# ExaScience/elprep

Measured on AMD Instinct MI355X. Metric: Mreads/s through sort+markdup+BQSR, 150bp PE, higher is better.
Workload: dtype u8/int32/int64 (integer path; float64 finalize on host)

## Files before the change

### elprep_amd/csrc/common.hpp

```cpp
#pragma once

#include <hip/hip_runtime.h>

#include <sched.h>

#include <cstdarg>
#include <cstdint>
#include <cstdio>
#include <cstring>
#include <map>
#include <mutex>
#include <string>
#include <vector>

#include "../../include/elprep_hip.h"
#include "../../include/elprep_hip_debug.h"
#include "derived.hpp"

namespace elp {

constexpr int WAVE = 64;

enum : uint16_t {
  F_MULTIPLE = 0x1, F_PROPER = 0x2, F_UNMAPPED = 0x4, F_NEXT_UNMAPPED = 0x8, F_REVERSED = 0x10, F_NEXT_REVERSED = 0x20,
  F_FIRST = 0x40, F_LAST = 0x80, F_SECONDARY = 0x100, F_QCFAILED = 0x200, F_DUPLICATE = 0x400, F_SUPPLEMENTARY = 0x800
};

enum : uint32_t { OP_M = 0, OP_I = 1, OP_D = 2, OP_N = 3, OP_S = 4, OP_H = 5, OP_P = 6, OP_EQ = 7, OP_X = 8 };

__host__ __device__ inline bool op_consumes_read(uint32_t op) { return op == OP_M || op == OP_I || op == OP_S || op == OP_EQ || op == OP_X; }
__host__ __device__ inline bool op_consumes_ref(uint32_t op) { return op == OP_M || op == OP_D || op == OP_N || op == OP_EQ || op == OP_X; }

size_t debug_guard_bytes();
void debug_guard_arm(void *p, size_t payload_bytes);
void debug_guard_release(void *p);
int debug_guard_check_all();

template <class T>
struct DVec {
  T *p = nullptr;
  size_t cap = 0;
  DVec() = default;
  DVec(const DVec &) = delete;
  DVec &operator=(const DVec &) = delete;
  ~DVec() { release(); }
  void release() {
    if (p) { debug_guard_release(p); (void)hipFree(p); }
    p = nullptr;
    cap = 0;
  }
  size_t bytes() const { return cap * sizeof(T); }
};

struct ProfPending {
  int name_id;
  hipEvent_t a, b;
};

}

struct elp_ctx {
  int device = 0;
  int n_cu = 256;
  hipStream_t stream = nullptr;
  std::string err;
  std::mutex stage_mu;

  bool have_header = false;
  int32_t n_ref = 0, n_rg = 0, n_lib = 0, n_cov = 0;
  std::vector<int32_t> h_ref_len;
  std::vector<uint16_t> h_rg_lib, h_rg_cov;
  elp::DVec<int32_t> ref_len;
  elp::DVec<uint16_t> rg_lib, rg_cov;
  bool dict_replaced = false;
  int32_t n_ref0 = 0;
  std::vector<int32_t> h_ref_len0;

  static constexpr uint64_t SEQ_FRONT = 16;
  uint64_t n = 0, qname_bytes = 0, cigar_ops = 0, seq_bytes = SEQ_FRONT, qual_bytes = 0;
  uint64_t n_sr = 0;
  uint64_t n_filtered = 0;
  elp::DVec<int32_t> refid, pos, next_refid, pnext, tlen;
  elp::DVec<uint16_t> flag, rgid, split;
  elp::DVec<uint8_t> mapq, has_sr;
  elp::DVec<uint32_t> l_seq;
  elp::DVec<uint64_t> qname_off, cigar_off, seq_off, qual_off;
  elp::DVec<uint8_t> qname, seq4, qual;
  elp::DVec<uint32_t> cigar;
  elp::DVec<uint64_t> stage_tmp;
  uint32_t max_qname_len = 0, max_l_seq = 0;
  uint32_t max_split = 0;
  uint32_t max_pos = 0;
  int key_bits = 64;

  elp::Derived derived;
  bool radix_check_pending = false;
  elp::DVec<uint32_t> adapt_err;
  unsigned long long adapt_qmask[2] = {0, 0};
  elp::DVec<uint2> apply_recs;
  int apply_recs_lmax = 0;
  unsigned long long qual_present[2] = {0, 0};
  elp::DVec<int32_t> upos, score;
  elp::DVec<uint64_t> qbounds;
  elp::DVec<uint64_t> key;
  elp::DVec<uint32_t> perm;
  elp::DVec<uint32_t> err_flag;
  elp::DVec<uint32_t> tile_first;
  void *h_pinned = nullptr;
  size_t h_pinned_cap = 0;
  elp::DVec<unsigned long long> radix_state;
  elp::DVec<uint32_t> radix_ticket;
  elp::DVec<unsigned long long> radix_hist;
  elp::DVec<uint32_t> scan_pool;
  elp::DVec<unsigned long long> xchg_hdr;
  elp::DVec<uint32_t> tie_live;
  elp::DVec<uint32_t> md_ctr;
  static constexpr uint32_t MAX_QNAME = 1000;
  static constexpr uint32_t TIE_LIVE_WORDS = 32;
  uint32_t radix_epoch = 0;
  uint32_t uniform_len = 0;

  elp::DVec<uint32_t> mate;
  elp::DVec<uint32_t> pair_win;

  std::vector<uint8_t *> h_ref_seq;
  std::vector<int64_t> h_ref_seq_len;
  std::vector<int32_t *> h_sites;
  std::vector<int64_t> h_n_sites;
  std::vector<uint8_t> ref_flags_dirty;
  std::vector<uint32_t *> h_site_idx;
  elp::DVec<uint8_t *> d_ref_seq;
  elp::DVec<int64_t> d_ref_seq_len;
  elp::DVec<int32_t *> d_sites;
  elp::DVec<uint32_t *> d_site_idx;
  elp::DVec<int64_t> d_n_sites;
  bool bqsr_ptrs_dirty = true;

  static constexpr size_t TABLES_TAIL = 4096;
  elp::DVec<unsigned long long> dev_tables;
  size_t tables_n = 0;
  int tables_max_cycle = 0;
  unsigned long long tables_quals[2] = {0, 0};
  elp::DVec<unsigned long long> tables_pack;
  elp::DVec<uint8_t> lut_rows_dev;
  void *comm = nullptr;
  bool comm_borrowed = false;
  int (*xport)(void *, int64_t *, size_t) = nullptr;
  void *xport_user = nullptr;
  int (*p2p)(void *, int, const void *, size_t, int, void *, size_t) = nullptr;
  void *p2p_user = nullptr;
  int group_rank = 0, group_world = 1;
  elp_ctx *group_owner = nullptr;
  std::vector<elp_ctx *> group_borrowers;

  elp::DVec<uint8_t> raw;
  elp::DVec<uint64_t> raw_off;
  uint64_t raw_n = 0, raw_bytes = 0;
  uint64_t max_raw_rec = 0;
  elp::DVec<uint8_t> rg_ids;
  elp::DVec<uint32_t> rg_ids_off;
  bool have_rg_ids = false;
  static constexpr size_t TAG_WORDS = 65536 / 32;
  bool tag_filter = false;
  std::vector<uint32_t> h_tag_drop;
  elp::DVec<uint32_t> tag_drop;
  bool replace_rg = false;
  std::string replace_rg_id;
  elp::DVec<uint8_t> replace_rg_dev;
  hipStream_t copy_stream = nullptr;
  elp::DVec<uint8_t> lut_dev;
  void *lut_pinned = nullptr;
  size_t lut_pinned_cap = 0;
  hipEvent_t lut_ev = nullptr;
  hipEvent_t apply_ev = nullptr;
  int lut_uploaded_cycle = 0;
  elp::DVec<uint32_t> lut_wk;
  bool dict_ready = false;
  bool dict_per_cov = false;
  int dict_qlo = 0, dict_nqi = 0, dict_lmax = 0, dict_cycle = 0, dict_ncov = 0;
  hipEvent_t tables_ev = nullptr;
  void *bounce[2] = {nullptr, nullptr};
  hipEvent_t bounce_ev[2] = {nullptr, nullptr};

  uint32_t *mail = nullptr;
  hipEvent_t mail_ev = nullptr;

  elp_ctx *side[2] = {nullptr, nullptr};
  hipEvent_t side_ev[2] = {nullptr, nullptr};
  hipEvent_t side_done[2] = {nullptr, nullptr};
  bool sort_ahead = false;
  uint64_t presort_n = 0;
  uint64_t *presort_ks = nullptr;
  int presort_idx_bits = 0;

  elp::DVec<uint16_t> snap_flag;
  elp::DVec<uint8_t> snap_qual;
  uint64_t snap_n = 0, snap_qual_bytes = 0;

  struct Tuning {
    int count_kernel = 0;
    int apply_kernel = 0;
    int count3_rlog = -1;
    int qual_hint = 0;
    int qual_hint_drop = -1;
    int pair_table_slots = 1 << 20;
    long long bgzf_piece = 1ll << 30;
    int bgzf_weak_guess = 0;
    int score_kernel = 0;
    int mate_path = 0;
    int radix_tile = 0;
    int sort_pairs = 0;
    int tie_rounds = 0;
    int exchange_piece = 0;
    int emit_pass = 0;
    long long bgzf_inflate_piece = 2ll << 30;
    int bgzf_copy_chunk = 0;
    int bgzf_tok_lds = 0;
    int bgzf_first_chunk_div = 4;
    int bgzf_fixed = 0;
    int bgzf_tok_fail_above = 0;
    int bgzf_stored = 0;
    int apply_wgs = 0;
    int presort_tile = 0;
    int side_priority = 0;
  } tune;

  elp::DVec<uint8_t> scratch[8];

  bool profiling = false;
  const char *prof_prefix = nullptr;
  std::vector<std::string> prof_names;
  std::map<std::string, int> prof_index;
  std::vector<uint64_t> prof_launches;
  std::vector<double> prof_ms;
  std::vector<elp::ProfPending> prof_pending;
};

namespace elp {

int set_error(elp_ctx *c, int code, const char *fmt, ...);
int prof_begin(elp_ctx *c, const char *name);
void prof_end(elp_ctx *c, int pending);
int prof_flush(elp_ctx *c);
struct ProfScope {
  elp_ctx *c;
  const char *saved;
  ProfScope(elp_ctx *ctx, const char *prefix) : c(ctx), saved(ctx->prof_prefix) { ctx->prof_prefix = prefix; }
  ~ProfScope() { c->prof_prefix = saved; }
};

#define ELP_HIP(ctx, call)                                                                             \
  do {                                                                                                 \
    hipError_t e__ = (call);                                                                           \
    if (e__ != hipSuccess)                                                                             \
      return elp::set_error((ctx), e__ == hipErrorOutOfMemory ? ELP_ERR_NOMEM : ELP_ERR_HIP, "%s failed: %s (%s:%d)", #call, \
                            hipGetErrorString(e__), __FILE__, __LINE__);                               \
  } while (0)

#define ELP_TRY(expr)            \
  do {                           \
    int rc__ = (expr);           \
    if (rc__ != 0) return rc__;  \
  } while (0)

bool sync_spin();
inline void spin_relax(unsigned &spins) {
  if (++spins < 4096u) {
#if defined(__x86_64__) || defined(__i386__)
    __builtin_ia32_pause();
#elif defined(__aarch64__)
    asm volatile("yield");
#endif
  } else {
    sched_yield();
  }
}
inline hipError_t stream_wait(hipStream_t st) {
  if (!sync_spin()) return hipStreamSynchronize(st);
  hipError_t e;
  unsigned spins = 0;
  while ((e = hipStreamQuery(st)) == hipErrorNotReady) spin_relax(spins);
  return e;
}
inline hipError_t event_wait(hipEvent_t ev) {
  if (!sync_spin()) return hipEventSynchronize(ev);
  hipError_t e;
  unsigned spins = 0;
  while ((e = hipEventQuery(ev)) == hipErrorNotReady) spin_relax(spins);
  return e;
}

int debug_poison();
bool debug_trace();

template <class T>
int ensure(elp_ctx *c, DVec<T> &v, size_t n, bool keep = false, size_t keep_elems = 0) {
  if (n <= v.cap) return 0;
  size_t ncap = keep ? (n + n / 2 + 16) : n;
  T *np = nullptr;
  ELP_HIP(c, hipMalloc((void **)&np, ncap * sizeof(T) + debug_guard_bytes()));
  if (debug_guard_bytes()) debug_guard_arm(np, ncap * sizeof(T));
  if (const int pz = debug_poison(); pz >= 0) {
    ELP_HIP(c, hipMemsetAsync(np, pz, ncap * sizeof(T), c->stream));
    ELP_HIP(c, elp::stream_wait(c->stream));
  }
  if (keep && v.p && keep_elems) {
    hipError_t e = hipMemcpyAsync(np, v.p, keep_elems * sizeof(T), hipMemcpyDeviceToDevice, c->stream);
    if (e == hipSuccess) e = elp::stream_wait(c->stream);
    if (e != hipSuccess) {
      (void)hipFree(np);
      return set_error(c, ELP_ERR_HIP, "device copy failed while growing a column: %s", hipGetErrorString(e));
    }
  }
  if (v.p) {
    (void)elp::stream_wait(c->stream);
    debug_guard_release(v.p);
    if (debug_poison() >= 0) { (void)hipMemsetAsync(v.p, 0xDD, v.cap * sizeof(T), c->stream); (void)elp::stream_wait(c->stream); }
    (void)hipFree(v.p);
  }
  v.p = np;
  v.cap = ncap;
  return 0;
}

template <class T>
int scratch(elp_ctx *c, int slot, size_t n, T **out) {
  ELP_TRY(ensure(c, c->scratch[slot], n * sizeof(T) + 256));
  *out = reinterpret_cast<T *>(c->scratch[slot].p);
  return 0;
}

#define ELP_LAUNCH(ctx, name, kernel, grid, block, shmem, ...)                              \
  do {                                                                                      \
    int pp__ = (ctx)->profiling ? elp::prof_begin((ctx), (name)) : -1;                      \
    if (elp::debug_trace()) fprintf(stderr, "[elp] %s\n", (name));                          \
    hipLaunchKernelGGL(kernel, grid, block, shmem, (ctx)->stream, __VA_ARGS__);             \
    if (pp__ >= 0) elp::prof_end((ctx), pp__);                                              \
    ELP_HIP((ctx), hipGetLastError());                                                      \
    if (elp::debug_trace()) ELP_HIP((ctx), elp::stream_wait((ctx)->stream));            \
  } while (0)

inline unsigned blocks_for(uint64_t n, unsigned per_block) { return (unsigned)((n + per_block - 1) / per_block); }

__device__ __forceinline__ uint64_t mix64(uint64_t x) {
  x ^= x >> 30; x *= 0xbf58476d1ce4e5b9ull; x ^= x >> 27; x *= 0x94d049bb133111ebull; x ^= x >> 31;
  return x;
}

__device__ __forceinline__ uint64_t load8(const uint8_t *__restrict__ p) {
  uint64_t w;
  __builtin_memcpy(&w, p, 8);
  return w;
}
__device__ __forceinline__ uint64_t low_bytes(uint64_t w, uint32_t nbytes) {
  return nbytes >= 8 ? w : (w & ((1ull << (8 * nbytes)) - 1ull));
}
__device__ inline int qname_cmp(const uint8_t *__restrict__ q, const uint64_t *__restrict__ off, uint32_t a, uint32_t b) {
  const uint64_t oa = off[a], ob = off[b];
  const uint32_t la = (uint32_t)(off[a + 1] - oa), lb = (uint32_t)(off[b + 1] - ob);
  const uint32_t m = la < lb ? la : lb;
  for (uint32_t i = 0; i < m; i += 8) {
    const uint32_t nb = m - i;
    const uint64_t wa = low_bytes(load8(q + oa + i), nb), wb = low_bytes(load8(q + ob + i), nb);
    if (wa != wb) {
      const uint64_t ba = __builtin_bswap64(wa), bb = __builtin_bswap64(wb);
      return ba < bb ? -1 : 1;
    }
  }
  return la < lb ? -1 : (la > lb ? 1 : 0);
}
__device__ inline bool qname_eq(const uint8_t *__restrict__ q, const uint64_t *__restrict__ off, uint32_t a, uint32_t b) {
  const uint64_t oa = off[a], ob = off[b];
  const uint32_t la = (uint32_t)(off[a + 1] - oa), lb = (uint32_t)(off[b + 1] - ob);
  if (la != lb) return false;
  uint64_t diff = 0;
  for (uint32_t i = 0; i < la && diff == 0; i += 32) {
    const uint64_t a0 = load8(q + oa + i), a1 = load8(q + oa + i + 8), a2 = load8(q + oa + i + 16), a3 = load8(q + oa + i + 24);
    const uint64_t b0 = load8(q + ob + i), b1 = load8(q + ob + i + 8), b2 = load8(q + ob + i + 16), b3 = load8(q + ob + i + 24);
    const uint32_t nb = la - i;
    diff |= low_bytes(a0 ^ b0, nb);
    diff |= nb > 8 ? low_bytes(a1 ^ b1, nb - 8) : 0ull;
    diff |= nb > 16 ? low_bytes(a2 ^ b2, nb - 16) : 0ull;
    diff |= nb > 24 ? low_bytes(a3 ^ b3, nb - 24) : 0ull;
  }
  return diff == 0;
}

__host__ __device__ inline uint16_t mod_flag(uint16_t flag) {
  if ((flag & F_MULTIPLE) == 0) flag &= (uint16_t) ~(F_NEXT_UNMAPPED | F_NEXT_REVERSED);
  if (flag & F_UNMAPPED) flag &= (uint16_t)~F_REVERSED;
  if (flag & F_NEXT_UNMAPPED) flag &= (uint16_t)~F_NEXT_REVERSED;
  return flag;
}

int radix_sort_pairs(elp_ctx *c, uint64_t *keys, uint32_t *vals, uint64_t *keys_tmp, uint32_t *vals_tmp, uint64_t n,
                     uint64_t **keys_out, uint32_t **vals_out);
int radix_sort_fused(elp_ctx *c, const uint64_t *keycol, uint64_t n, int key_bits, int idx_bits, uint64_t *buf0, uint64_t *buf1, uint64_t **out);
struct RadixBounds {
  uint32_t *start = nullptr, *nend = nullptr;
  uint32_t mask = 0;
  int shift = 0;
};
int radix_sort_pairs_low(elp_ctx *c, uint64_t *keys, uint32_t *vals, uint64_t *keys_tmp, uint32_t *vals_tmp, uint64_t n, int ndigits,
                         uint64_t **keys_out, uint32_t **vals_out, const uint64_t *first_src = nullptr, bool identity_vals = false,
                         const uint32_t *n_dev = nullptr , RadixBounds bnd = RadixBounds{});
int exclusive_scan_u32(elp_ctx *c, const uint32_t *in, uint32_t *out, uint64_t n, uint32_t *total_host );
int ensure_adapted(elp_ctx *c, bool check_quals = true);
int ensure_keys(elp_ctx *c);
int adapt_begin(elp_ctx *c, int *pos_bits);
int adapt_scores(elp_ctx *c);
int mailbox(elp_ctx *c);
int side_lane(elp_ctx *c, int lane, elp_ctx **out);
int side_join(elp_ctx *c, int lane);
int sort_presort(elp_ctx *c);
void prof_merge_side(elp_ctx *c);
constexpr int ADAPT_WORDS = 6;
void adapt_note(elp_ctx *c, const uint32_t *words );
int adapt_quality_error(elp_ctx *c);
int ensure_uniform_len(elp_ctx *c);
int ensure_qual_present(elp_ctx *c, bool exact = false);
int fetch_err(elp_ctx *c, uint32_t *words );
int radix_check(elp_ctx *c);
void group_release(elp_ctx *c);
int group_sendrecv(elp_ctx *c, int send_peer, const void *send_dev, size_t send_bytes, int recv_peer, void *recv_dev, size_t recv_bytes);
int tables_written(elp_ctx *c);
int stage_reserve(elp_ctx *c, uint64_t n, uint64_t qb, uint64_t co, uint64_t sb, uint64_t lb);
int merge_refuses_queryname(elp_ctx *groups, const char *who);
int merge_spread_slots(elp_ctx *groups, elp_ctx *spread, uint64_t **slots_out);
int stage_recode_seq(elp_ctx *c, uint64_t from, uint64_t bytes);
inline void clear_run_settings(elp_ctx *c) { c->tag_filter = false; c->replace_rg = false; c->replace_rg_id.clear(); }
inline bool same_replace_rg(const elp_ctx *a, const elp_ctx *b) { return a->replace_rg == b->replace_rg && a->replace_rg_id == b->replace_rg_id; }
int install_dictionary(elp_ctx *c, int32_t n_ref, const int32_t *ref_len);
int staging_refused_after_replace(elp_ctx *c, const char *who);
int stage_bam_columns(elp_ctx *c, uint32_t n_rec, uint64_t piece_bytes, uint64_t raw_end, uint64_t max_raw_rec, uint16_t split_id);
uint64_t bgzf_framed_size(uint64_t n_bytes);
int bgzf_frame(elp_ctx *c, const uint8_t *raw, uint64_t n_bytes, uint8_t *out);
int bgzf_deflate(elp_ctx *c, const uint8_t *raw, uint64_t n_bytes, uint8_t *out, uint64_t *out_bytes);

}
```

### elprep_amd/csrc/ctx.hip

```cpp
#include "common.hpp"

namespace elp {

namespace {
constexpr size_t GUARD = 4096;
constexpr uint8_t GUARD_BYTE = 0xC3;
std::mutex guard_mu;
std::map<void *, size_t> guard_of;
int guard_check_one(void *p, size_t payload) {
  uint8_t host[GUARD];
  if (hipDeviceSynchronize() != hipSuccess || hipMemcpy(host, static_cast<uint8_t *>(p) + payload, GUARD, hipMemcpyDeviceToHost) != hipSuccess) return 0;
  for (size_t k = 0; k < GUARD; k++)
    if (host[k] != GUARD_BYTE) {
      fprintf(stderr, "[elp] ELP_DEBUG_GUARD: byte %zu behind the end of a %zu-byte device buffer was overwritten (0x%02x)\n", k, payload, host[k]);
      return 1;
    }
  return 0;
}
}
size_t debug_guard_bytes() {
  static const size_t v = [] { const char *e = getenv("ELP_DEBUG_GUARD"); return (e && *e && *e != '0') ? GUARD : (size_t)0; }();
  return v;
}
void debug_guard_arm(void *p, size_t payload) {
  (void)hipMemset(static_cast<uint8_t *>(p) + payload, GUARD_BYTE, GUARD);
  (void)hipDeviceSynchronize();
  std::lock_guard<std::mutex> lk(guard_mu);
  guard_of[p] = payload;
}
void debug_guard_release(void *p) {
  if (!debug_guard_bytes()) return;
  size_t payload = 0;
  {
    std::lock_guard<std::mutex> lk(guard_mu);
    auto it = guard_of.find(p);
    if (it == guard_of.end()) return;
    payload = it->second;
    guard_of.erase(it);
  }
  if (guard_check_one(p, payload)) abort();
}
int debug_guard_check_all() {
  if (!debug_guard_bytes()) return 0;
  std::lock_guard<std::mutex> lk(guard_mu);
  int bad = 0;
  for (auto &kv : guard_of) bad += guard_check_one(kv.first, kv.second);
  return bad;
}

bool sync_spin() {
  static const bool v = [] { const char *e = getenv("ELP_SYNC_SPIN"); return !(e && *e == '0'); }();
  return v;
}
bool debug_trace() {
  static const bool v = [] { const char *e = getenv("ELP_DEBUG_TRACE"); return e && *e && *e != '0'; }();
  return v;
}
int debug_poison() {
  static const int v = [] {
    const char *e = getenv("ELP_DEBUG_POISON");
    return (e && *e) ? (int)(strtol(e, nullptr, 0) & 0xFF) : -1;
  }();
  return v;
}


int set_error(elp_ctx *c, int code, const char *fmt, ...) {
  char buf[1024];
  va_list ap;
  va_start(ap, fmt);
  vsnprintf(buf, sizeof buf, fmt, ap);
  va_end(ap);
  if (c) c->err = buf;
  return code;
}

int prof_begin(elp_ctx *c, const char *name0) {
  const std::string name = c->prof_prefix ? std::string(c->prof_prefix) + name0 : std::string(name0);
  auto it = c->prof_index.find(name);
  int id;
  if (it == c->prof_index.end()) {
    id = (int)c->prof_names.size();
    c->prof_names.push_back(name);
    c->prof_index[name] = id;
    c->prof_launches.push_back(0);
    c->prof_ms.push_back(0.0);
  } else {
    id = it->second;
  }
  ProfPending p;
  p.name_id = id;
  if (hipEventCreate(&p.a) != hipSuccess) return -1;
  if (hipEventCreate(&p.b) != hipSuccess) { (void)hipEventDestroy(p.a); return -1; }
  (void)hipEventRecord(p.a, c->stream);
  c->prof_pending.push_back(p);
  return (int)c->prof_pending.size() - 1;
}
void prof_end(elp_ctx *c, int pending) { (void)hipEventRecord(c->prof_pending[pending].b, c->stream); }
int prof_flush(elp_ctx *c) {
  if (c->prof_pending.empty()) return 0;
  ELP_HIP(c, elp::stream_wait(c->stream));
  for (auto &p : c->prof_pending) {
    float ms = 0.f;
    if (hipEventElapsedTime(&ms, p.a, p.b) == hipSuccess) {
      c->prof_ms[p.name_id] += ms;
      c->prof_launches[p.name_id] += 1;
    }
    (void)hipEventDestroy(p.a);
    (void)hipEventDestroy(p.b);
  }
  c->prof_pending.clear();
  return 0;
}

__global__ void k_rebase_offsets(const uint64_t *__restrict__ src, uint64_t *__restrict__ dst, uint64_t n_plus_1, uint64_t base,
                                 uint64_t src0) {
  uint64_t i = (uint64_t)blockIdx.x * blockDim.x + threadIdx.x;
  if (i < n_plus_1) dst[i] = src[i] - src0 + base;
}

__device__ __forceinline__ uint32_t recode_byte(uint32_t b) {
  constexpr uint64_t TAB = 0x8888888388828108ull;
  return (uint32_t)((TAB >> (4 * (b >> 4))) & 15u) | ((uint32_t)((TAB >> (4 * (b & 15u))) & 15u) << 4);
}
__global__ __launch_bounds__(256) void k_recode_seq(uint8_t *__restrict__ seq, uint64_t nbytes) {
  const uint64_t i = ((uint64_t)blockIdx.x * blockDim.x + threadIdx.x) * 16;
  if (i >= nbytes) return;
  if (i + 16 <= nbytes) {
    uint32_t w[4];
    __builtin_memcpy(w, seq + i, 16);
#pragma unroll
    for (int k = 0; k < 4; k++) {
      const uint32_t x = w[k];
      w[k] = recode_byte(x & 0xFFu) | (recode_byte((x >> 8) & 0xFFu) << 8) | (recode_byte((x >> 16) & 0xFFu) << 16) | (recode_byte(x >> 24) << 24);
    }
    __builtin_memcpy(seq + i, w, 16);
  } else {
    for (uint64_t k = i; k < nbytes; k++) seq[k] = (uint8_t)recode_byte(seq[k]);
  }
}

int stage_recode_seq(elp_ctx *c, uint64_t from, uint64_t bytes) {
  hipLaunchKernelGGL(k_recode_seq, dim3(blocks_for((bytes + 15) / 16, 256)), dim3(256), 0, c->stream, c->seq4.p + from, bytes);
  ELP_HIP(c, hipGetLastError());
  return 0;
}

int fetch_err(elp_ctx *c, uint32_t *words) {
  ELP_HIP(c, hipMemcpyAsync(words, c->err_flag.p, 4 * sizeof(uint32_t), hipMemcpyDeviceToHost, c->stream));
  ELP_HIP(c, elp::stream_wait(c->stream));
  c->radix_check_pending = false;
  if (words[0] & 256u) {
    const uint32_t w0 = words[0] & ~256u;
    ELP_HIP(c, hipMemcpyAsync(c->err_flag.p, &w0, 4, hipMemcpyHostToDevice, c->stream));
    ELP_HIP(c, elp::stream_wait(c->stream));
    c->derived.radix_timed_out();
    return set_error(c, ELP_ERR_HIP, "radix sort: tile look-back timed out");
  }
  return 0;
}
int mailbox(elp_ctx *c) {
  if (!c->mail) ELP_HIP(c, hipHostMalloc((void **)&c->mail, 1024 * sizeof(uint32_t), hipHostMallocDefault));
  if (!c->mail_ev) ELP_HIP(c, hipEventCreateWithFlags(&c->mail_ev, hipEventDisableTiming));
  return 0;
}
int side_lane(elp_ctx *c, int lane, elp_ctx **out) {
  if (!c->side[lane]) {
    elp_ctx *s = new elp_ctx();
    s->device = c->device;
    s->n_cu = c->n_cu;
    int prio_lo = 0, prio_hi = 0;
    (void)hipDeviceGetStreamPriorityRange(&prio_lo, &prio_hi);
    const hipError_t se = c->tune.side_priority != 1 ? hipStreamCreateWithFlags(&s->stream, hipStreamNonBlocking)
                                                     : hipStreamCreateWithPriority(&s->stream, hipStreamNonBlocking, prio_hi);
    if (se != hipSuccess || ensure(s, s->err_flag, 4) != 0 ||
        hipMemsetAsync(s->err_flag.p, 0, 16, s->stream) != hipSuccess) {
      if (s->stream) (void)hipStreamDestroy(s->stream);
      delete s;
      return set_error(c, ELP_ERR_HIP, "the side lane's stream could not be made");
    }
    c->side[lane] = s;
  }
  if (!c->side_ev[lane]) ELP_HIP(c, hipEventCreateWithFlags(&c->side_ev[lane], hipEventDisableTiming));
  if (!c->side_done[lane]) ELP_HIP(c, hipEventCreateWithFlags(&c->side_done[lane], hipEventDisableTiming));
  ELP_HIP(c, hipEventRecord(c->side_ev[lane], c->stream));
  ELP_HIP(c, hipStreamWaitEvent(c->side[lane]->stream, c->side_ev[lane], 0));
  c->side[lane]->profiling = c->profiling;
  c->side[lane]->tune = c->tune;
  *out = c->side[lane];
  return 0;
}
int side_join(elp_ctx *c, int lane) {
  ELP_HIP(c, hipEventRecord(c->side_done[lane], c->side[lane]->stream));
  ELP_HIP(c, hipStreamWaitEvent(c->stream, c->side_done[lane], 0));
  return 0;
}
void prof_merge_side(elp_ctx *c) {
  for (int lane = 0; lane < 2; lane++) {
    elp_ctx *s = c->side[lane];
    if (!s) continue;
    (void)prof_flush(s);
    for (size_t k = 0; k < s->prof_names.size(); k++) {
      if (!s->prof_launches[k]) continue;
      auto it = c->prof_index.find(s->prof_names[k]);
      int id;
      if (it == c->prof_index.end()) {
        id = (int)c->prof_names.size();
        c->prof_names.push_back(s->prof_names[k]);
        c->prof_index[s->prof_names[k]] = id;
        c->prof_launches.push_back(0);
        c->prof_ms.push_back(0.0);
      } else {
        id = it->second;
      }
      c->prof_launches[id] += s->prof_launches[k];
      c->prof_ms[id] += s->prof_ms[k];
      s->prof_launches[k] = 0;
      s->prof_ms[k] = 0.0;
    }
  }
}
int radix_check(elp_ctx *c) {
  if (!c->radix_check_pending) return 0;
  uint32_t e[4];
  return fetch_err(c, e);
}

int release_bqsr_inputs(elp_ctx *c) {
  ELP_HIP(c, elp::stream_wait(c->stream));
  for (auto &p : c->h_ref_seq) if (p) { (void)hipFree(p); p = nullptr; }
  for (auto &p : c->h_sites) if (p) { (void)hipFree(p); p = nullptr; }
  for (auto &p : c->h_site_idx) if (p) { (void)hipFree(p); p = nullptr; }
  for (auto &v : c->h_ref_seq_len) v = 0;
  for (auto &v : c->h_n_sites) v = 0;
  c->bqsr_ptrs_dirty = true;
  return 0;
}
int install_dictionary(elp_ctx *c, int32_t n_ref, const int32_t *ref_len) {
  ELP_TRY(ensure(c, c->ref_len, (size_t)n_ref + 1));
  ELP_TRY(release_bqsr_inputs(c));
  const std::vector<int32_t> len(ref_len, ref_len + n_ref);
  c->n_ref = n_ref;
  c->h_ref_len = len;
  if (n_ref) ELP_HIP(c, hipMemcpyAsync(c->ref_len.p, c->h_ref_len.data(), (size_t)n_ref * sizeof(int32_t), hipMemcpyHostToDevice, c->stream));
  ELP_HIP(c, elp::stream_wait(c->stream));
  c->h_ref_seq.assign((size_t)n_ref, nullptr);
  c->h_ref_seq_len.assign((size_t)n_ref, 0);
  c->h_sites.assign((size_t)n_ref, nullptr);
  c->h_site_idx.assign((size_t)n_ref, nullptr);
  c->h_n_sites.assign((size_t)n_ref, 0);
  c->ref_flags_dirty.assign((size_t)n_ref, 0);
  c->bqsr_ptrs_dirty = true;
  return 0;
}
int staging_refused_after_replace(elp_ctx *c, const char *who) {
  return set_error(c, ELP_ERR_ARG, "%s: the reference dictionary was replaced (elp_replace_reference_dictionary): the staged refids are the new "
                   "dictionary's, the header's are the old one's; call elp_reset or elp_set_header first", who);
}

}

using namespace elp;

extern "C" {

int elp_debug_check_guards(void) { return elp::debug_guard_check_all(); }


int elp_create(int device_ordinal, elp_ctx **out) {
  if (!out) return ELP_ERR_ARG;
  *out = nullptr;
  int ndev = 0;
  if (hipGetDeviceCount(&ndev) != hipSuccess || ndev <= 0) return ELP_ERR_HIP;
  if (device_ordinal < 0 || device_ordinal >= ndev) return ELP_ERR_ARG;
  if (hipSetDevice(device_ordinal) != hipSuccess) return ELP_ERR_HIP;
  hipDeviceProp_t prop;
  if (hipGetDeviceProperties(&prop, device_ordinal) != hipSuccess) return ELP_ERR_HIP;
  if (strncmp(prop.gcnArchName, "gfx950", 6) != 0) return ELP_ERR_UNSUPPORTED;
  elp_ctx *c = new elp_ctx();
  c->device = device_ordinal;
  c->n_cu = prop.multiProcessorCount > 0 ? prop.multiProcessorCount : 256;
  if (hipStreamCreateWithFlags(&c->stream, hipStreamNonBlocking) != hipSuccess) { delete c; return ELP_ERR_HIP; }
  if (ensure(c, c->err_flag, 4) != 0 || hipMemsetAsync(c->err_flag.p, 0, 16, c->stream) != hipSuccess) { delete c; return ELP_ERR_HIP; }
  *out = c;
  return ELP_OK;
}

void elp_destroy(elp_ctx *c) {
  if (!c) return;
  (void)hipSetDevice(c->device);
  (void)elp::stream_wait(c->stream);
  for (auto &p : c->prof_pending) { (void)hipEventDestroy(p.a); (void)hipEventDestroy(p.b); }
  if (c->lut_pinned) (void)hipHostFree(c->lut_pinned);
  if (c->lut_ev) (void)hipEventDestroy(c->lut_ev);
  if (c->apply_ev) (void)hipEventDestroy(c->apply_ev);
  for (auto p : c->h_ref_seq) if (p) (void)hipFree(p);
  for (auto p : c->h_sites) if (p) (void)hipFree(p);
  for (auto p : c->h_site_idx) if (p) (void)hipFree(p);
  if (c->h_pinned) (void)hipHostFree(c->h_pinned);
  for (int lane = 0; lane < 2; lane++) {
    if (c->side[lane]) {
      (void)elp::stream_wait(c->side[lane]->stream);
      for (auto &p : c->side[lane]->prof_pending) { (void)hipEventDestroy(p.a); (void)hipEventDestroy(p.b); }
      (void)hipStreamDestroy(c->side[lane]->stream);
      delete c->side[lane];
      c->side[lane] = nullptr;
    }
    if (c->side_ev[lane]) (void)hipEventDestroy(c->side_ev[lane]);
    if (c->side_done[lane]) (void)hipEventDestroy(c->side_done[lane]);
  }
  if (c->mail) (void)hipHostFree(c->mail);
  if (c->mail_ev) (void)hipEventDestroy(c->mail_ev);
  for (int k = 0; k < 2; k++) {
    if (c->bounce[k]) (void)hipHostFree(c->bounce[k]);
    if (c->bounce_ev[k]) (void)hipEventDestroy(c->bounce_ev[k]);
  }
  if (c->copy_stream) (void)hipStreamDestroy(c->copy_stream);
  if (c->tables_ev) (void)hipEventDestroy(c->tables_ev);
  group_release(c);
  (void)hipStreamDestroy(c->stream);
  delete c;
}

const char *elp_last_error(const elp_ctx *c) { return c ? c->err.c_str() : "null context"; }

int elp_sync(elp_ctx *c) {
  if (!c) return ELP_ERR_ARG;
  if (c->radix_check_pending) return radix_check(c);
  ELP_HIP(c, elp::stream_wait(c->stream));
  return 0;
}

void *elp_stream(elp_ctx *c) { return c ? (void *)c->stream : nullptr; }

int elp_set_header(elp_ctx *c, const elp_header *h) {
  if (!c || !h || h->n_ref < 0 || h->n_rg < 0 || (h->n_ref && !h->ref_len) || (h->n_rg && (!h->rg_lib || !h->rg_cov)))
    return set_error(c, ELP_ERR_ARG, "elp_set_header: bad arguments");
  ELP_HIP(c, hipSetDevice(c->device));
  if (c->dict_replaced) ELP_TRY(release_bqsr_inputs(c));
  c->n_ref = h->n_ref; c->n_rg = h->n_rg; c->n_lib = h->n_lib; c->n_cov = h->n_cov;
  c->derived.header_changed();
  clear_run_settings(c);
  c->h_ref_len.assign(h->ref_len, h->ref_len + h->n_ref);
  c->n_ref0 = h->n_ref;
  c->h_ref_len0 = c->h_ref_len;
  c->dict_replaced = false;
  c->h_rg_lib.assign(h->rg_lib, h->rg_lib + h->n_rg);
  c->h_rg_cov.assign(h->rg_cov, h->rg_cov + h->n_rg);
  for (int i = 0; i < h->n_rg; i++) {
    if (c->h_rg_lib[i] != ELP_NIL16 && c->h_rg_lib[i] >= h->n_lib) return set_error(c, ELP_ERR_ARG, "rg_lib[%d] out of range", i);
    if (c->h_rg_cov[i] >= h->n_cov) return set_error(c, ELP_ERR_ARG, "rg_cov[%d] out of range", i);
  }
  ELP_TRY(ensure(c, c->ref_len, (size_t)h->n_ref + 1));
  ELP_TRY(ensure(c, c->rg_lib, (size_t)h->n_rg + 1));
  ELP_TRY(ensure(c, c->rg_cov, (size_t)h->n_rg + 1));
  if (h->n_ref) ELP_HIP(c, hipMemcpyAsync(c->ref_len.p, h->ref_len, h->n_ref * sizeof(int32_t), hipMemcpyHostToDevice, c->stream));
  if (h->n_rg) {
    ELP_HIP(c, hipMemcpyAsync(c->rg_lib.p, h->rg_lib, h->n_rg * sizeof(uint16_t), hipMemcpyHostToDevice, c->stream));
    ELP_HIP(c, hipMemcpyAsync(c->rg_cov.p, h->rg_cov, h->n_rg * sizeof(uint16_t), hipMemcpyHostToDevice, c->stream));
  }
  ELP_HIP(c, elp::stream_wait(c->stream));
  c->h_ref_seq.resize(h->n_ref, nullptr);
  c->h_ref_seq_len.resize(h->n_ref, 0);
  c->h_sites.resize(h->n_ref, nullptr);
  c->h_site_idx.resize(h->n_ref, nullptr);
  c->h_n_sites.resize(h->n_ref, 0);
  c->ref_flags_dirty.assign(h->n_ref, 0);
  c->bqsr_ptrs_dirty = true;
  c->have_header = true;
  return 0;
}

}
namespace elp {
int stage_reserve(elp_ctx *c, uint64_t n, uint64_t qb, uint64_t co, uint64_t sb, uint64_t lb) {
  bool keep = c->n > 0;
  ELP_TRY(ensure(c, c->refid, n, keep, c->n));
  ELP_TRY(ensure(c, c->pos, n, keep, c->n));
  ELP_TRY(ensure(c, c->next_refid, n, keep, c->n));
  ELP_TRY(ensure(c, c->pnext, n, keep, c->n));
  ELP_TRY(ensure(c, c->tlen, n, keep, c->n));
  ELP_TRY(ensure(c, c->flag, n, keep, c->n));
  ELP_TRY(ensure(c, c->rgid, n, keep, c->n));
  ELP_TRY(ensure(c, c->split, n, keep, c->n));
  ELP_TRY(ensure(c, c->mapq, n, keep, c->n));
  ELP_TRY(ensure(c, c->has_sr, n, keep, c->n));
  ELP_TRY(ensure(c, c->l_seq, n, keep, c->n));
  ELP_TRY(ensure(c, c->qname_off, n + 1, keep, c->n + 1));
  ELP_TRY(ensure(c, c->cigar_off, n + 1, keep, c->n + 1));
  ELP_TRY(ensure(c, c->seq_off, n + 1, keep, c->n + 1));
  ELP_TRY(ensure(c, c->qual_off, n + 1, keep, c->n + 1));
  ELP_TRY(ensure(c, c->qname, qb + 64, keep, c->qname_bytes));
  ELP_TRY(ensure(c, c->cigar, co + 4, keep, c->cigar_ops));
  ELP_TRY(ensure(c, c->seq4, sb + 32, keep, c->seq_bytes));
  ELP_TRY(ensure(c, c->qual, lb + 32, keep, c->qual_bytes));
  return 0;
}
}
extern "C" {

int elp_reserve(elp_ctx *c, uint64_t n, uint64_t qb, uint64_t co, uint64_t sb, uint64_t lb) {
  if (!c) return ELP_ERR_ARG;
  std::lock_guard<std::mutex> g(c->stage_mu);
  ELP_HIP(c, hipSetDevice(c->device));
  return stage_reserve(c, n, qb, co, sb + elp_ctx::SEQ_FRONT, lb);
}

int elp_reset(elp_ctx *c) {
  if (!c) return ELP_ERR_ARG;
  std::lock_guard<std::mutex> g(c->stage_mu);
  c->n = c->qname_bytes = c->cigar_ops = c->qual_bytes = 0;
  c->seq_bytes = elp_ctx::SEQ_FRONT;
  c->n_sr = 0;
  c->n_filtered = 0;
  c->raw_n = c->raw_bytes = 0;
  c->max_raw_rec = 0;
  c->max_split = 0;
  c->max_qname_len = c->max_l_seq = 0;
  c->max_pos = 0;
  c->derived.records_changed();
  clear_run_settings(c);
  if (c->dict_replaced) {
    ELP_HIP(c, hipSetDevice(c->device));
    ELP_TRY(install_dictionary(c, c->n_ref0, c->h_ref_len0.data()));
    c->derived.header_changed();
    c->dict_replaced = false;
  }
  return 0;
}

uint64_t elp_num_records(const elp_ctx *c) { return c ? c->n : 0; }
uint64_t elp_num_sorted(const elp_ctx *c) { return c ? c->n - c->n_sr : 0; }
uint64_t elp_num_qual_bytes(const elp_ctx *c) { return c ? c->qual_bytes : 0; }

int elp_stage(elp_ctx *c, const elp_batch *b) {
  if (!c || !b) return ELP_ERR_ARG;
  std::lock_guard<std::mutex> g(c->stage_mu);
  ELP_HIP(c, hipSetDevice(c->device));
  if (!c->have_header) return set_error(c, ELP_ERR_ARG, "elp_stage: call elp_set_header first");
  if (c->dict_replaced) return staging_refused_after_replace(c, "elp_stage");
  uint64_t n = b->n;
  if (n == 0) return 0;
  if (c->n + n > 0xFFFFFFF0ull) return set_error(c, ELP_ERR_UNSUPPORTED, "more than 2^32-16 records per context");
  uint64_t q0 = b->qname_off[0], c0 = b->cigar_off[0], s0 = b->seq_off[0], l0 = b->qual_off[0];
  uint64_t qb = b->qname_off[n] - q0, co = b->cigar_off[n] - c0, sb = b->seq_off[n] - s0, lb = b->qual_off[n] - l0;
  ELP_TRY(stage_reserve(c, c->n + n, c->qname_bytes + qb, c->cigar_ops + co, c->seq_bytes + sb, c->qual_bytes + lb));
  hipStream_t st = c->stream;
  uint64_t at = c->n;
#define H2D(dst, src, cnt, T) ELP_HIP(c, hipMemcpyAsync((dst), (src), (cnt) * sizeof(T), hipMemcpyHostToDevice, st))
  if (lb) H2D(c->qual.p + c->qual_bytes, b->qual + l0, lb, uint8_t);
  if (sb) {
    H2D(c->seq4.p + c->seq_bytes, b->seq4 + s0, sb, uint8_t);
    hipLaunchKernelGGL(k_recode_seq, dim3(blocks_for((sb + 15) / 16, 256)), dim3(256), 0, st, c->seq4.p + c->seq_bytes, sb);
    ELP_HIP(c, hipGetLastError());
  }
  if (qb) H2D(c->qname.p + c->qname_bytes, b->qname + q0, qb, uint8_t);
  if (co) H2D(c->cigar.p + c->cigar_ops, b->cigar + c0, co, uint32_t);
  H2D(c->refid.p + at, b->refid, n, int32_t);
  H2D(c->pos.p + at, b->pos, n, int32_t);
  H2D(c->next_refid.p + at, b->next_refid, n, int32_t);
  H2D(c->pnext.p + at, b->pnext, n, int32_t);
  H2D(c->tlen.p + at, b->tlen, n, int32_t);
  H2D(c->flag.p + at, b->flag, n, uint16_t);
  H2D(c->rgid.p + at, b->rgid, n, uint16_t);
  if (b->split) H2D(c->split.p + at, b->split, n, uint16_t);
  else ELP_HIP(c, hipMemsetAsync(c->split.p + at, 0, n * sizeof(uint16_t), st));
  H2D(c->mapq.p + at, b->mapq, n, uint8_t);
  H2D(c->l_seq.p + at, b->l_seq, n, uint32_t);
  if (b->has_sr) H2D(c->has_sr.p + at, b->has_sr, n, uint8_t);
  else ELP_HIP(c, hipMemsetAsync(c->has_sr.p + at, 0, n, st));
  ELP_TRY(ensure(c, c->stage_tmp, 4 * (n + 1)));
  unsigned blk = 256, grd = blocks_for(n + 1, blk);
  struct { const uint64_t *src; uint64_t *dst; uint64_t base; } offs[4] = {
      {b->qname_off, c->qname_off.p + at, c->qname_bytes}, {b->cigar_off, c->cigar_off.p + at, c->cigar_ops},
      {b->seq_off, c->seq_off.p + at, c->seq_bytes}, {b->qual_off, c->qual_off.p + at, c->qual_bytes}};
  for (int k = 0; k < 4; k++) H2D(c->stage_tmp.p + (size_t)k * (n + 1), offs[k].src, n + 1, uint64_t);
  for (int k = 0; k < 4; k++) {
    hipLaunchKernelGGL(k_rebase_offsets, dim3(grd), dim3(blk), 0, st, (const uint64_t *)(c->stage_tmp.p + (size_t)k * (n + 1)), offs[k].dst, n + 1, offs[k].base,
                       offs[k].src[0]);
    ELP_HIP(c, hipGetLastError());
  }
#undef H2D
  uint64_t n_sr = 0;
  uint32_t max_split = c->max_split;
  uint32_t max_qname_len = c->max_qname_len, max_l_seq = c->max_l_seq, max_pos = c->max_pos;
  int scan_rc = 0;
  for (uint64_t i = 0; i < n && !scan_rc; i++) {
    uint64_t ql = b->qname_off[i + 1] - b->qname_off[i];
    if (ql > elp_ctx::MAX_QNAME) scan_rc = set_error(c, ELP_ERR_UNSUPPORTED, "record %llu: QNAME of %llu bytes (limit %u)", (unsigned long long)i, (unsigned long long)ql, elp_ctx::MAX_QNAME);
    if (b->has_sr && b->has_sr[i]) n_sr++;
    if (b->split && b->split[i] > max_split) max_split = b->split[i];
    if (ql > max_qname_len) max_qname_len = (uint32_t)ql;
    if (b->l_seq[i] > max_l_seq) max_l_seq = b->l_seq[i];
    if ((uint32_t)b->pos[i] > max_pos) max_pos = (uint32_t)b->pos[i];
    if (b->qual_off[i + 1] - b->qual_off[i] > 0x3FFFFFull || b->l_seq[i] > 0x3FFFFFu)
      scan_rc = set_error(c, ELP_ERR_UNSUPPORTED, "record %llu: more than 4194303 bases", (unsigned long long)i);
    if (b->rgid[i] != ELP_NIL16 && b->rgid[i] >= c->n_rg) scan_rc = set_error(c, ELP_ERR_ARG, "record %llu: rgid %u not in header", (unsigned long long)i, b->rgid[i]);
    if (b->refid[i] >= c->n_ref) scan_rc = set_error(c, ELP_ERR_ARG, "record %llu: refid %d not in header", (unsigned long long)i, b->refid[i]);
  }
  if (scan_rc) { (void)elp::stream_wait(st); return scan_rc; }
  ELP_HIP(c, elp::stream_wait(st));
  c->n += n; c->qname_bytes += qb; c->cigar_ops += co; c->seq_bytes += sb; c->qual_bytes += lb;
  c->n_sr += n_sr;
  c->max_split = max_split;
  c->max_qname_len = max_qname_len; c->max_l_seq = max_l_seq; c->max_pos = max_pos;
  c->derived.records_changed();
  return 0;
}

int elp_stage_columns(elp_ctx *c, uint64_t n, const int32_t *refid, const int32_t *pos, const int32_t *next_refid, const int32_t *pnext, const int32_t *tlen,
                      const uint16_t *flag, const uint8_t *mapq, const uint16_t *rgid, const uint8_t *has_sr, const uint32_t *l_seq,
                      const uint64_t *qname_off, const uint8_t *qname, const uint64_t *cigar_off, const uint32_t *cigar, const uint64_t *seq_off,
                      const uint8_t *seq4, const uint64_t *qual_off, const uint8_t *qual, const uint16_t *split) {
  if (!c) return ELP_ERR_ARG;
  if (n && (!refid || !pos || !next_refid || !pnext || !tlen || !flag || !mapq || !rgid || !l_seq || !qname_off || !cigar_off || !seq_off || !qual_off))
    return set_error(c, ELP_ERR_ARG, "elp_stage_columns: a required column is NULL");
  elp_batch b;
  b.n = n; b.refid = refid; b.pos = pos; b.next_refid = next_refid; b.pnext = pnext; b.tlen = tlen; b.flag = flag; b.mapq = mapq; b.rgid = rgid;
  b.has_sr = has_sr; b.l_seq = l_seq; b.qname_off = qname_off; b.qname = qname; b.cigar_off = cigar_off; b.cigar = cigar; b.seq_off = seq_off;
  b.seq4 = seq4; b.qual_off = qual_off; b.qual = qual; b.split = split;
  return elp_stage(c, &b);
}

int elp_set_header_columns(elp_ctx *c, int32_t n_ref, const int32_t *ref_len, int32_t n_rg, const uint16_t *rg_lib, const uint16_t *rg_cov, int32_t n_lib,
                           int32_t n_cov) {
  elp_header h;
  h.n_ref = n_ref; h.ref_len = ref_len; h.n_rg = n_rg; h.rg_lib = rg_lib; h.rg_cov = rg_cov; h.n_lib = n_lib; h.n_cov = n_cov;
  return elp_set_header(c, &h);
}

static int d2h(elp_ctx *c, void *dst, const void *src, size_t bytes) {
  if (!bytes) return 0;
  ELP_HIP(c, hipSetDevice(c->device));
  ELP_HIP(c, hipMemcpyAsync(dst, src, bytes, hipMemcpyDeviceToHost, c->stream));
  ELP_HIP(c, elp::stream_wait(c->stream));
  return 0;
}

int elp_get_permutation(elp_ctx *c, uint32_t *out) {
  if (!c || (!out && c->n)) return ELP_ERR_ARG;
  if (!c->derived.sorted) return set_error(c, ELP_ERR_ARG, "elp_get_permutation: call elp_sort_coordinate or elp_sort_queryname first");
  ELP_TRY(radix_check(c));
  return d2h(c, out, c->perm.p, c->n * sizeof(uint32_t));
}
int elp_get_flags(elp_ctx *c, uint16_t *out) {
  if (!c || (!out && c->n)) return ELP_ERR_ARG;
  ELP_TRY(radix_check(c));
  return d2h(c, out, c->flag.p, c->n * sizeof(uint16_t));
}
int elp_get_adapted(elp_ctx *c, int32_t *upos, int32_t *score) {
  if (!c) return ELP_ERR_ARG;
  ELP_TRY(ensure_adapted(c));
  if (upos) ELP_TRY(d2h(c, upos, c->upos.p, c->n * sizeof(int32_t)));
  if (score) ELP_TRY(d2h(c, score, c->score.p, c->n * sizeof(int32_t)));
  return 0;
}
int elp_get_qual(elp_ctx *c, uint8_t *out) {
  if (!c || (!out && c->qual_bytes)) return ELP_ERR_ARG;
  return d2h(c, out, c->qual.p, c->qual_bytes);
}

int elp_snapshot(elp_ctx *c) {
  if (!c) return ELP_ERR_ARG;
  ELP_HIP(c, hipSetDevice(c->device));
  ELP_TRY(ensure(c, c->snap_flag, c->n + 1));
  ELP_TRY(ensure(c, c->snap_qual, c->qual_bytes + 16));
  if (c->n) ELP_HIP(c, hipMemcpyAsync(c->snap_flag.p, c->flag.p, c->n * sizeof(uint16_t), hipMemcpyDeviceToDevice, c->stream));
  if (c->qual_bytes) ELP_HIP(c, hipMemcpyAsync(c->snap_qual.p, c->qual.p, c->qual_bytes, hipMemcpyDeviceToDevice, c->stream));
  c->snap_n = c->n;
  c->snap_qual_bytes = c->qual_bytes;
  c->derived.have_snapshot = true;
  return 0;
}
int elp_rollback(elp_ctx *c) {
  if (!c) return ELP_ERR_ARG;
  if (!c->derived.have_snapshot || c->snap_n != c->n || c->snap_qual_bytes != c->qual_bytes)
    return set_error(c, ELP_ERR_ARG, "elp_rollback: no snapshot of the current record set");
  ELP_HIP(c, hipSetDevice(c->device));
  if (c->n) ELP_HIP(c, hipMemcpyAsync(c->flag.p, c->snap_flag.p, c->n * sizeof(uint16_t), hipMemcpyDeviceToDevice, c->stream));
  if (c->qual_bytes) ELP_HIP(c, hipMemcpyAsync(c->qual.p, c->snap_qual.p, c->qual_bytes, hipMemcpyDeviceToDevice, c->stream));
  c->derived.flag_qual_restored();
  return 0;
}

int elp_set_tuning(elp_ctx *c, const char *key, int64_t value) {
  if (!c || !key) return ELP_ERR_ARG;
  const std::string k(key);
  const int v = (int)value;
  if (k == "count_kernel") c->tune.count_kernel = v;
  else if (k == "apply_kernel") c->tune.apply_kernel = v;
  else if (k == "bgzf_piece") { if (value < 1) return set_error(c, ELP_ERR_ARG, "elp_set_tuning: bgzf_piece must be positive"); c->tune.bgzf_piece = value; }
  else if (k == "bgzf_weak_guess") c->tune.bgzf_weak_guess = v;
  else if (k == "score_kernel") { c->tune.score_kernel = v; c->derived.score_tuning_changed(); }
  else if (k == "count3_rlog") c->tune.count3_rlog = v;
  else if (k == "qual_hint") { c->tune.qual_hint = v; c->derived.hint_tuning_changed(); }
  else if (k == "qual_hint_drop") { c->tune.qual_hint_drop = v; c->derived.hint_tuning_changed(); }
  else if (k == "pair_table_slots") {
    if (v == 0) { c->tune.pair_table_slots = 1 << 20; return 0; }
    if (v < 2 || v > (1 << 20) || (v & (v - 1))) return set_error(c, ELP_ERR_ARG, "elp_set_tuning: pair_table_slots must be a power of two >= 2");
    c->tune.pair_table_slots = v;
  } else if (k == "mate_path") {
    if (value != 0 && value != 2) return set_error(c, ELP_ERR_ARG, "elp_set_tuning: mate_path is 0 (the library decides) or 2 (every candidate through the table)");
    c->tune.mate_path = v;
  } else if (k == "tie_rounds") c->tune.tie_rounds = v;
  else if (k == "radix_tile") c->tune.radix_tile = v;
  else if (k == "sort_pairs") c->tune.sort_pairs = v;
  else if (k == "exchange_piece") c->tune.exchange_piece = v;
  else if (k == "emit_pass") c->tune.emit_pass = v;
  else if (k == "bgzf_stored") c->tune.bgzf_stored = v;
  else if (k == "bgzf_tok_fail_above") c->tune.bgzf_tok_fail_above = v;
  else if (k == "bgzf_fixed") c->tune.bgzf_fixed = v;
  else if (k == "bgzf_first_chunk_div") c->tune.bgzf_first_chunk_div = v;
  else if (k == "bgzf_tok_lds") c->tune.bgzf_tok_lds = v;
  else if (k == "bgzf_copy_chunk") c->tune.bgzf_copy_chunk = v;
  else if (k == "bgzf_inflate_piece") { if (value < 1) return set_error(c, ELP_ERR_ARG, "elp_set_tuning: bgzf_inflate_piece must be positive"); c->tune.bgzf_inflate_piece = value; }
  else if (k == "md_fused" || k == "bgzf_inflate") {
    if (value != 0) return set_error(c, ELP_ERR_ARG, "elp_set_tuning: key '%s' is retired (only 0 is accepted)", key);
  } else if (k == "apply_wgs") c->tune.apply_wgs = v;
  else if (k == "presort_tile") c->tune.presort_tile = v;
  else if (k == "side_priority") c->tune.side_priority = v;
  else return set_error(c, ELP_ERR_ARG, "elp_set_tuning: unknown key '%s'", key);
  return 0;
}

int elp_profile_enable(elp_ctx *c, int on) {
  if (!c) return ELP_ERR_ARG;
  if (!on) { ELP_TRY(prof_flush(c)); prof_merge_side(c); }
  c->profiling = on != 0;
  for (int lane = 0; lane < 2; lane++)
    if (c->side[lane]) c->side[lane]->profiling = c->profiling;
  return 0;
}
int elp_profile_reset(elp_ctx *c) {
  if (!c) return ELP_ERR_ARG;
  ELP_TRY(prof_flush(c));
  prof_merge_side(c);
  for (auto &v : c->prof_launches) v = 0;
  for (auto &v : c->prof_ms) v = 0.0;
  return 0;
}
int elp_profile_count(elp_ctx *c) {
  if (!c) return ELP_ERR_ARG;
  if (prof_flush(c) != 0) return ELP_ERR_HIP;
  prof_merge_side(c);
  return (int)c->prof_names.size();
}
int elp_profile_get(elp_ctx *c, int index, const char **name, uint64_t *launches, double *total_ms) {
  if (!c || index < 0 || index >= (int)c->prof_names.size()) return ELP_ERR_ARG;
  if (name) *name = c->prof_names[index].c_str();
  if (launches) *launches = c->prof_launches[index];
  if (total_ms) *total_ms = c->prof_ms[index];
  return 0;
}

}
```

### elprep_amd/csrc/radix.hip

```cpp
#include "common.hpp"

namespace elp {

__device__ __forceinline__ uint32_t wave_incl_scan(uint32_t v) {
  const int lane = threadIdx.x & 63;
#pragma unroll
  for (int d = 1; d < 64; d <<= 1) {
    uint32_t t = __shfl_up(v, d, 64);
    if (lane >= d) v += t;
  }
  return v;
}

__device__ __forceinline__ uint32_t block_excl_scan_256(uint32_t v, uint32_t *total, uint32_t *lds ) {
  const int lane = threadIdx.x & 63, w = threadIdx.x >> 6;
  uint32_t inc = wave_incl_scan(v);
  if (lane == 63) lds[w] = inc;
  __syncthreads();
  uint32_t base = 0, tot = 0;
#pragma unroll
  for (int i = 0; i < 4; i++) {
    uint32_t s = lds[i];
    if (i < w) base += s;
    tot += s;
  }
  __syncthreads();
  *total = tot;
  return base + inc - v;
}

constexpr int SCAN_ITEMS = 8;
constexpr int SCAN_TILE = 256 * SCAN_ITEMS;

__global__ __launch_bounds__(256) void k_scan_reduce(const uint32_t *__restrict__ in, uint32_t *__restrict__ sums, uint64_t n) {
  __shared__ uint32_t lds[8];
  uint64_t base = (uint64_t)blockIdx.x * SCAN_TILE + (uint64_t)threadIdx.x * SCAN_ITEMS;
  uint32_t s = 0;
#pragma unroll
  for (int i = 0; i < SCAN_ITEMS; i++)
    if (base + i < n) s += in[base + i];
  uint32_t tot;
  (void)block_excl_scan_256(s, &tot, lds);
  if (threadIdx.x == 0) sums[blockIdx.x] = tot;
}

__global__ __launch_bounds__(256) void k_scan_down(const uint32_t *__restrict__ in, uint32_t *__restrict__ out,
                                                   const uint32_t *__restrict__ block_base, uint64_t n) {
  __shared__ uint32_t lds[8];
  uint64_t base = (uint64_t)blockIdx.x * SCAN_TILE + (uint64_t)threadIdx.x * SCAN_ITEMS;
  uint32_t v[SCAN_ITEMS];
  uint32_t s = 0;
#pragma unroll
  for (int i = 0; i < SCAN_ITEMS; i++) {
    v[i] = (base + i < n) ? in[base + i] : 0u;
    s += v[i];
  }
  uint32_t tot;
  uint32_t ex = block_excl_scan_256(s, &tot, lds) + (block_base ? block_base[blockIdx.x] : 0u);
#pragma unroll
  for (int i = 0; i < SCAN_ITEMS; i++) {
    if (base + i < n) out[base + i] = ex;
    ex += v[i];
  }
}

static int scan_levels(elp_ctx *c, const uint32_t *in, uint32_t *out, uint64_t n, uint32_t *total_dev) {
  if (n == 0) {
    if (total_dev) ELP_HIP(c, hipMemsetAsync(total_dev, 0, 4, c->stream));
    return 0;
  }
  std::vector<uint64_t> cnt;
  cnt.push_back(n);
  while (true) {
    uint64_t nb = (cnt.back() + SCAN_TILE - 1) / SCAN_TILE;
    cnt.push_back(nb);
    if (nb <= 1) break;
  }
  size_t need = 0;
  for (size_t k = 1; k < cnt.size(); k++) need += cnt[k] + 4;
  uint32_t *pool;
  ELP_TRY(ensure(c, c->scan_pool, need + 16));
  pool = c->scan_pool.p;
  std::vector<uint32_t *> sums(cnt.size(), nullptr);
  size_t off = 0;
  for (size_t k = 1; k < cnt.size(); k++) { sums[k] = pool + off; off += cnt[k] + 4; }
  const uint32_t *src = in;
  for (size_t k = 0; k + 1 < cnt.size(); k++) {
    ELP_LAUNCH(c, "scan_reduce", k_scan_reduce, dim3((unsigned)cnt[k + 1]), dim3(256), 0, src, sums[k + 1], cnt[k]);
    src = sums[k + 1];
  }
  size_t top = cnt.size() - 1;
  if (total_dev) ELP_HIP(c, hipMemcpyAsync(total_dev, sums[top], 4, hipMemcpyDeviceToDevice, c->stream));
  ELP_HIP(c, hipMemsetAsync(sums[top], 0, 4, c->stream));
  for (size_t k = top - 1; k >= 1; k--) {
    ELP_LAUNCH(c, "scan_down", k_scan_down, dim3((unsigned)cnt[k + 1]), dim3(256), 0, (const uint32_t *)sums[k], sums[k],
               (const uint32_t *)sums[k + 1], cnt[k]);
  }
  ELP_LAUNCH(c, "scan_down", k_scan_down, dim3((unsigned)cnt[1]), dim3(256), 0, in, out, (const uint32_t *)sums[1], n);
  return 0;
}

int exclusive_scan_u32(elp_ctx *c, const uint32_t *in, uint32_t *out, uint64_t n, uint32_t *total_host) {
  uint32_t *tot_dev = nullptr;
  if (total_host) tot_dev = c->err_flag.p + 3;
  ELP_TRY(scan_levels(c, in, out, n, tot_dev));
  if (total_host) {
    ELP_HIP(c, hipMemcpyAsync(total_host, tot_dev, 4, hipMemcpyDeviceToHost, c->stream));
    ELP_HIP(c, elp::stream_wait(c->stream));
    ELP_HIP(c, hipMemsetAsync(tot_dev, 0, 4, c->stream));
  }
  return 0;
}

constexpr int RS_THREADS = 256;
constexpr int RS_ITEMS = 16;
constexpr int RS_TILE = RS_THREADS * RS_ITEMS;

template <int ND>
__global__ __launch_bounds__(256) void k_radix_hist_all(const uint64_t *__restrict__ keys, uint64_t n, unsigned long long *__restrict__ ghist ,
                                                        const uint32_t *__restrict__ n_dev) {
  __shared__ uint32_t h[8][256];
  if (n_dev) n = *n_dev;
  for (int i = threadIdx.x; i < 8 * 256; i += 256) (&h[0][0])[i] = 0;
  __syncthreads();
  for (uint64_t i = (uint64_t)blockIdx.x * 256 + threadIdx.x; i < n; i += (uint64_t)gridDim.x * 256) {
    uint64_t k = keys[i];
    const unsigned long long act = __ballot(1);
    const int first = __ffsll((long long)act) - 1;
#pragma unroll
    for (int d = 0; d < ND; d++) {
      uint32_t dg = (uint32_t)(k >> (8 * d)) & 0xFF;
      uint32_t d0 = __shfl(dg, first, 64);
      if (__all(dg == d0)) {
        if ((int)(threadIdx.x & 63) == first) atomicAdd(&h[d][d0], (uint32_t)__popcll(act));
      } else {
        atomicAdd(&h[d][dg], 1u);
      }
    }
  }
  __syncthreads();
  for (int i = threadIdx.x; i < ND * 256; i += 256) {
    uint32_t v = (&h[0][0])[i];
    if (v) atomicAdd(&ghist[i], (unsigned long long)v);
  }
}

constexpr unsigned long long RS_AGG = 1ull << 32, RS_INCL = 2ull << 32;

template <int THREADS, bool PAIRS>
__global__ __launch_bounds__(THREADS, THREADS >= 512 ? 4 : 1) void k_radix_scatter_t(const uint64_t *__restrict__ keys, const uint32_t *__restrict__ vals,
                                                              uint64_t *__restrict__ keys_out, uint32_t *__restrict__ vals_out, uint64_t n,
                                                              int shift, const unsigned long long *__restrict__ ghist ,
                                                              unsigned long long *state, uint32_t epoch, uint32_t *ticket,
                                                              uint32_t *err, const uint32_t *__restrict__ n_dev, int fuse, RadixBounds bnd) {
  constexpr int WAVES = THREADS / 64, TILE = THREADS * RS_ITEMS;
  __shared__ uint32_t cnt[WAVES][256];
  __shared__ uint32_t gbase[256];
  __shared__ uint32_t scan_lds[16];
  extern __shared__ __attribute__((aligned(16))) uint64_t sbuf_dyn[];
  __shared__ uint64_t sbuf_static[THREADS == 256 ? RS_TILE : 1];
  uint64_t *const sbuf = THREADS == 256 ? sbuf_static : sbuf_dyn;
  __shared__ uint32_t my_tile;
  const int lane = threadIdx.x & 63, w = threadIdx.x >> 6;
  if (threadIdx.x == 0) my_tile = atomicAdd(ticket, 1u);
  for (int i = threadIdx.x; i < WAVES * 256; i += THREADS) (&cnt[0][0])[i] = 0;
  __syncthreads();
  const uint32_t tile = my_tile;
  const uint64_t tbase = (uint64_t)tile * TILE;
  if (n_dev) {
    n = *n_dev;
    if (tbase >= n) return;
  }
  const uint64_t wbase = tbase + (uint64_t)w * (64 * RS_ITEMS);
  const uint32_t tile_n = (uint32_t)((n - tbase) < (uint64_t)TILE ? (n - tbase) : (uint64_t)TILE);
  uint64_t k[RS_ITEMS];
  uint32_t v[PAIRS ? RS_ITEMS : 1];
  uint32_t pos[RS_ITEMS];
  const unsigned long long lt_mask = (1ull << lane) - 1ull;
#pragma unroll
  for (int r = 0; r < RS_ITEMS; r++) {
    uint64_t i = wbase + (uint64_t)r * 64 + lane;
    bool valid = i < n;
    k[r] = valid ? keys[i] : ~0ull;
    if (!PAIRS && fuse && valid) k[r] = (k[r] << fuse) | i;
    if (PAIRS) v[r] = valid ? (vals ? vals[i] : (uint32_t)i) : 0u;
    uint32_t d = (uint32_t)(k[r] >> shift) & 0xFF;
    unsigned long long peers = __ballot(valid);
    peers = valid ? peers : ~peers;
#pragma unroll
    for (int b = 0; b < 8; b++) {
      unsigned long long m = __ballot((d >> b) & 1);
      peers &= ((d >> b) & 1) ? m : ~m;
    }
    uint32_t before = (uint32_t)__popcll(peers & lt_mask);
    int leader = __ffsll((long long)peers) - 1;
    uint32_t old = 0;
    if (valid && lane == leader) {
      old = cnt[w][d];
      cnt[w][d] = old + (uint32_t)__popcll(peers);
    }
    old = __shfl(old, leader, 64);
    pos[r] = old + before;
  }
  __syncthreads();
  uint32_t tot = 0, tstart;
  const unsigned long long tag = (unsigned long long)epoch << 34;
  const bool owner = THREADS == 256 || threadIdx.x < 256;
  const uint32_t dg = THREADS == 256 ? threadIdx.x : (threadIdx.x & 255u);
  unsigned long long *mine = state + (size_t)tile * 256 + dg;
  {
    if (owner) {
#pragma unroll
      for (int i = 0; i < WAVES; i++) tot += cnt[i][dg];
      __hip_atomic_store(mine, tag | (tile == 0 ? RS_INCL : RS_AGG) | tot, __ATOMIC_RELAXED, __HIP_MEMORY_SCOPE_AGENT);
    }
    uint32_t all;
    tstart = block_excl_scan_256(tot, &all, scan_lds);
    if (owner) {
      uint32_t run = tstart;
#pragma unroll
      for (int i = 0; i < WAVES; i++) {
        uint32_t t = cnt[i][dg];
        cnt[i][dg] = run;
        run += t;
      }
    }
  }
  __syncthreads();
#pragma unroll
  for (int r = 0; r < RS_ITEMS; r++) {
    uint64_t i = wbase + (uint64_t)r * 64 + lane;
    if (i < n) {
      uint32_t d = (uint32_t)(k[r] >> shift) & 0xFF;
      pos[r] += cnt[w][d];
      sbuf[pos[r]] = k[r];
    }
  }
  {
    uint32_t dall;
    const uint32_t dbase = block_excl_scan_256(owner ? (uint32_t)ghist[dg] : 0u, &dall, scan_lds);
    uint32_t prefix = 0;
    if (tile != 0 && owner) {
      constexpr int LB = 8;
      uint32_t back = 1, spins = 0;
      bool done = false;
      while (!done) {
        unsigned long long v[LB];
#pragma unroll
        for (int i = 0; i < LB; i++) {
          const uint32_t b = back + (uint32_t)i;
          v[i] = b <= tile ? __hip_atomic_load(mine - (size_t)b * 256, __ATOMIC_RELAXED, __HIP_MEMORY_SCOPE_AGENT) : (tag | RS_INCL);
        }
#pragma unroll
        for (int i = 0; i < LB; i++) {
          if (done || (v[i] >> 34) != epoch) break;
          prefix += (uint32_t)v[i];
          back++;
          done = (v[i] & RS_INCL) != 0;
        }
        if (!done) {
          __builtin_amdgcn_s_sleep(1);
          if (++spins == (1u << 22)) { atomicOr(err, 256u); break; }
        }
      }
      __hip_atomic_store(mine, tag | RS_INCL | (prefix + tot), __ATOMIC_RELAXED, __HIP_MEMORY_SCOPE_AGENT);
    }
    if (owner) gbase[dg] = dbase + prefix - tstart;
  }
  __syncthreads();
  uint32_t dst[RS_ITEMS];
#pragma unroll
  for (int r = 0; r < RS_ITEMS; r++) {
    const uint32_t j = (uint32_t)r * THREADS + threadIdx.x;
    if (j < tile_n) {
      const uint64_t key = sbuf[j];
      dst[r] = gbase[(uint32_t)(key >> shift) & 0xFF] + j;
      keys_out[dst[r]] = key;
      if (PAIRS && bnd.start) {
        const uint32_t b = ((uint32_t)key & bnd.mask) >> bnd.shift;
        const bool first = j == 0 || (((uint32_t)sbuf[j - 1] & bnd.mask) >> bnd.shift) != b;
        const bool last = j + 1 == tile_n || (((uint32_t)sbuf[j + 1] & bnd.mask) >> bnd.shift) != b;
        if (first) atomicMin(&bnd.start[b], dst[r]);
        if (last) atomicMin(&bnd.nend[b], ~(dst[r] + 1u));
      }
    }
  }
  if (!PAIRS) return;
  __syncthreads();
  uint32_t *sval = reinterpret_cast<uint32_t *>(sbuf);
#pragma unroll
  for (int r = 0; r < RS_ITEMS; r++) {
    uint64_t i = wbase + (uint64_t)r * 64 + lane;
    if (i < n) sval[pos[r]] = v[PAIRS ? r : 0];
  }
  __syncthreads();
#pragma unroll
  for (int r = 0; r < RS_ITEMS; r++) {
    const uint32_t j = (uint32_t)r * THREADS + threadIdx.x;
    if (j < tile_n) vals_out[dst[r]] = sval[j];
  }
}

static int radix_pass_setup(elp_ctx *c, uint32_t ntiles) {
  if ((size_t)ntiles * 256 > c->radix_state.cap) {
    ELP_TRY(ensure(c, c->radix_state, (size_t)ntiles * 256));
    ELP_HIP(c, hipMemsetAsync(c->radix_state.p, 0, c->radix_state.cap * sizeof(unsigned long long), c->stream));
    c->radix_epoch = 0;
  }
  return 0;
}
static int radix_next_epoch(elp_ctx *c) {
  if (++c->radix_epoch >= (1u << 30)) {
    ELP_HIP(c, hipMemsetAsync(c->radix_state.p, 0, c->radix_state.cap * sizeof(unsigned long long), c->stream));
    c->radix_epoch = 1;
  }
  return 0;
}

static int radix_tile_shift(const elp_ctx *c, uint64_t n) {
  if (c->tune.radix_tile >= 1 && c->tune.radix_tile <= 3) return c->tune.radix_tile - 1;
  return n >= (16ull << 20) ? 2 : n >= (4ull << 20) ? 1 : 0;
}
static bool radix_big_tiles(const elp_ctx *c, uint64_t n) { return radix_tile_shift(c, n) == 1; }
static uint32_t radix_tiles(const elp_ctx *c, uint64_t n) {
  const uint64_t tile = (uint64_t)RS_TILE << radix_tile_shift(c, n);
  return (uint32_t)((n + tile - 1) / tile);
}
template <bool PAIRS>
static int radix_scatter_launch_t(elp_ctx *c, uint64_t n, const uint64_t *kin, const uint32_t *vin, uint64_t *kdst, uint32_t *vdst, int shift,
                                  const unsigned long long *ghist, uint32_t *ticket, const uint32_t *n_dev, int fuse, RadixBounds bnd = RadixBounds{}) {
  const uint32_t ntiles = radix_tiles(c, n);
  const int ts = radix_tile_shift(c, n);
  if (ts == 2) {
    const size_t dyn = (size_t)4 * RS_TILE * sizeof(uint64_t);
    ELP_HIP(c, hipFuncSetAttribute(reinterpret_cast<const void *>(&k_radix_scatter_t<1024, PAIRS>), hipFuncAttributeMaxDynamicSharedMemorySize, (int)dyn));
    ELP_LAUNCH(c, "radix_scatter", (k_radix_scatter_t<1024, PAIRS>), dim3(ntiles), dim3(1024), dyn, kin, vin, kdst, vdst, n, shift, ghist, c->radix_state.p,
               c->radix_epoch, ticket, c->err_flag.p, n_dev, fuse, bnd);
  } else if (ts == 1) {
    const size_t dyn = (size_t)2 * RS_TILE * sizeof(uint64_t);
    ELP_HIP(c, hipFuncSetAttribute(reinterpret_cast<const void *>(&k_radix_scatter_t<512, PAIRS>), hipFuncAttributeMaxDynamicSharedMemorySize, (int)dyn));
    ELP_LAUNCH(c, "radix_scatter", (k_radix_scatter_t<512, PAIRS>), dim3(ntiles), dim3(512), dyn, kin, vin, kdst, vdst, n, shift, ghist, c->radix_state.p,
               c->radix_epoch, ticket, c->err_flag.p, n_dev, fuse, bnd);
  } else {
    ELP_LAUNCH(c, "radix_scatter", (k_radix_scatter_t<256, PAIRS>), dim3(ntiles), dim3(256), 0, kin, vin, kdst, vdst, n, shift, ghist, c->radix_state.p,
               c->radix_epoch, ticket, c->err_flag.p, n_dev, fuse, bnd);
  }
  return 0;
}
static int radix_scatter_launch(elp_ctx *c, uint64_t n, const uint64_t *kin, const uint32_t *vin, uint64_t *kdst, uint32_t *vdst, int shift,
                                const unsigned long long *ghist, uint32_t *ticket, const uint32_t *n_dev, RadixBounds bnd = RadixBounds{}) {
  return radix_scatter_launch_t<true>(c, n, kin, vin, kdst, vdst, shift, ghist, ticket, n_dev, 0, bnd);
}

int radix_sort_fused(elp_ctx *c, const uint64_t *keycol, uint64_t n, int key_bits, int idx_bits, uint64_t *buf0, uint64_t *buf1, uint64_t **out) {
  if (n >= 0xFFFFFFFFull || key_bits + idx_bits > 64 || key_bits < 1 || idx_bits < 1) return set_error(c, ELP_ERR_UNSUPPORTED, "radix sort: bad size");
  const int ndigits = (key_bits + 7) / 8;
  unsigned long long *ghist;
  ELP_TRY(ensure(c, c->radix_hist, 8 * 256 + 4));
  ghist = c->radix_hist.p;
  ELP_HIP(c, hipMemsetAsync(ghist, 0, (8 * 256 + 4) * sizeof(unsigned long long), c->stream));
  uint32_t *ticket = reinterpret_cast<uint32_t *>(ghist + 8 * 256);
  const unsigned hb = (unsigned)std::min<uint64_t>((n + 255) / 256, 2048);
  if (ndigits <= 2) ELP_LAUNCH(c, "radix_hist_all", k_radix_hist_all<2>, dim3(hb), dim3(256), 0, keycol, n, ghist, (const uint32_t *)nullptr);
  else if (ndigits <= 4) ELP_LAUNCH(c, "radix_hist_all", k_radix_hist_all<4>, dim3(hb), dim3(256), 0, keycol, n, ghist, (const uint32_t *)nullptr);
  else ELP_LAUNCH(c, "radix_hist_all", k_radix_hist_all<8>, dim3(hb), dim3(256), 0, keycol, n, ghist, (const uint32_t *)nullptr);
  ELP_TRY(radix_pass_setup(c, radix_tiles(c, n)));
  uint64_t *src = buf1, *dst = buf0;
  for (int d = 0; d < ndigits; d++) {
    ELP_TRY(radix_next_epoch(c));
    ELP_TRY(radix_scatter_launch_t<false>(c, n, d == 0 ? keycol : src, nullptr, dst, nullptr, idx_bits + 8 * d, (const unsigned long long *)(ghist + d * 256),
                                          ticket + d, nullptr, d == 0 ? idx_bits : 0));
    std::swap(src, dst);
  }
  *out = src;
  return 0;
}

int radix_sort_pairs_low(elp_ctx *c, uint64_t *keys, uint32_t *vals, uint64_t *keys_tmp, uint32_t *vals_tmp, uint64_t n, int ndigits,
                         uint64_t **keys_out, uint32_t **vals_out, const uint64_t *first_src, bool identity_vals, const uint32_t *n_dev, RadixBounds bnd) {
  *keys_out = keys;
  *vals_out = vals;
  if ((ndigits <= 0 || (n < 2 && !n_dev)) && !first_src && !identity_vals) return 0;
  if (ndigits <= 0) ndigits = 1;
  if (n >= 0xFFFFFFFFull || ndigits > 8) return set_error(c, ELP_ERR_UNSUPPORTED, "radix sort: bad size");
  unsigned long long *ghist;
  ELP_TRY(ensure(c, c->radix_hist, 8 * 256 + 4));
  ghist = c->radix_hist.p;
  ELP_HIP(c, hipMemsetAsync(ghist, 0, (8 * 256 + 4) * sizeof(unsigned long long), c->stream));
  uint32_t *ticket = reinterpret_cast<uint32_t *>(ghist + 8 * 256);
  const unsigned hb = (unsigned)std::min<uint64_t>((n + 255) / 256, 2048);
  if (ndigits <= 2) ELP_LAUNCH(c, "radix_hist_all", k_radix_hist_all<2>, dim3(hb), dim3(256), 0, (const uint64_t *)(first_src ? first_src : keys), n, ghist, n_dev);
  else if (ndigits <= 4) ELP_LAUNCH(c, "radix_hist_all", k_radix_hist_all<4>, dim3(hb), dim3(256), 0, (const uint64_t *)(first_src ? first_src : keys), n, ghist, n_dev);
  else ELP_LAUNCH(c, "radix_hist_all", k_radix_hist_all<8>, dim3(hb), dim3(256), 0, (const uint64_t *)(first_src ? first_src : keys), n, ghist, n_dev);
  ELP_TRY(radix_pass_setup(c, radix_tiles(c, n)));
  uint64_t *ksrc = keys, *kdst = keys_tmp;
  uint32_t *vsrc = vals, *vdst = vals_tmp;
  for (int d = 0; d < ndigits; d++) {
    ELP_TRY(radix_next_epoch(c));
    const uint64_t *kin = (d == 0 && first_src) ? first_src : ksrc;
    const uint32_t *vin = (d == 0 && identity_vals) ? nullptr : vsrc;
    ELP_TRY(radix_scatter_launch(c, n, kin, vin, kdst, vdst, 8 * d, (const unsigned long long *)(ghist + d * 256), ticket + d, n_dev,
                                 d == ndigits - 1 ? bnd : RadixBounds{}));
    std::swap(ksrc, kdst);
    std::swap(vsrc, vdst);
  }
  *keys_out = ksrc;
  *vals_out = vsrc;
  return 0;
}

int radix_sort_pairs(elp_ctx *c, uint64_t *keys, uint32_t *vals, uint64_t *keys_tmp, uint32_t *vals_tmp, uint64_t n, uint64_t **keys_out,
                     uint32_t **vals_out) {
  *keys_out = keys;
  *vals_out = vals;
  if (n < 2) return 0;
  if (n >= 0xFFFFFFFFull) return set_error(c, ELP_ERR_UNSUPPORTED, "radix sort: more than 2^32-1 elements");
  unsigned long long *ghist;
  ELP_TRY(ensure(c, c->radix_hist, 8 * 256 + 4));
  ghist = c->radix_hist.p;
  ELP_HIP(c, hipMemsetAsync(ghist, 0, (8 * 256 + 4) * sizeof(unsigned long long), c->stream));
  uint32_t *ticket = reinterpret_cast<uint32_t *>(ghist + 8 * 256);
  unsigned hb = (unsigned)std::min<uint64_t>((n + 255) / 256, 2048);
  ELP_LAUNCH(c, "radix_hist_all", k_radix_hist_all<8>, dim3(hb), dim3(256), 0, (const uint64_t *)keys, n, ghist, (const uint32_t *)nullptr);
  unsigned long long hh[8 * 256];
  ELP_HIP(c, hipMemcpyAsync(hh, ghist, sizeof hh, hipMemcpyDeviceToHost, c->stream));
  ELP_HIP(c, elp::stream_wait(c->stream));
  ELP_TRY(radix_pass_setup(c, radix_tiles(c, n)));
  uint64_t *ksrc = keys, *kdst = keys_tmp;
  uint32_t *vsrc = vals, *vdst = vals_tmp;
  for (int d = 0; d < 8; d++) {
    bool live = true;
    for (int b = 0; b < 256; b++)
      if (hh[d * 256 + b] == n) { live = false; break; }
    if (!live) continue;
    ELP_TRY(radix_next_epoch(c));
    ELP_TRY(radix_scatter_launch(c, n, ksrc, vsrc, kdst, vdst, 8 * d, (const unsigned long long *)(ghist + d * 256), ticket + d, nullptr));
    std::swap(ksrc, kdst);
    std::swap(vsrc, vdst);
  }
  *keys_out = ksrc;
  *vals_out = vsrc;
  return 0;
}

}
```

### elprep_amd/csrc/sort.hip

```cpp
#include <cstdlib>

#include "apply_rec.hpp"
#include "common.hpp"
#include "flat.hpp"

namespace elp {

constexpr int TIE_SMALL = 48;

__global__ __launch_bounds__(256) void k_adapt_fixed(uint64_t n, const int32_t *__restrict__ pos, const int32_t *__restrict__ refid,
                                                     const uint16_t *__restrict__ flag, const uint64_t *__restrict__ cigar_off,
                                                     const uint32_t *__restrict__ cigar, int32_t *__restrict__ upos, int32_t *__restrict__ score,
                                                     uint64_t *__restrict__ key, uint32_t n_ref, int pos_bits,
                                                     const uint8_t *__restrict__ has_sr) {
  uint64_t i = (uint64_t)blockIdx.x * blockDim.x + threadIdx.x;
  if (i >= n) return;
  const uint16_t f = flag[i];
  const int32_t p = pos[i];
  const int32_t r = refid[i];
  const uint64_t ru = has_sr[i] ? (uint64_t)n_ref + 1 : (r < 0 ? (uint64_t)n_ref : (uint64_t)(uint32_t)r);
  key[i] = (ru << (pos_bits + 1)) | ((uint64_t)(uint32_t)p << 1) | ((f & F_REVERSED) ? 1ull : 0ull);
  int32_t up = 0;
  if ((f & (F_UNMAPPED | F_SECONDARY | F_SUPPLEMENTARY)) == 0) {
    const uint64_t c0 = cigar_off[i], c1 = cigar_off[i + 1];
    up = p;
    if (c1 > c0) {
      if (f & F_REVERSED) {
        int32_t clipped = 1;
        up--;
        for (uint64_t k = c1; k-- > c0;) {
          const uint32_t c = cigar[k];
          const uint32_t op = c & 0xF;
          const int32_t isclip = (op == OP_S || op == OP_H) ? 1 : 0;
          const int32_t isref = op_consumes_ref(op) ? 1 : 0;
          clipped *= isclip;
          up += (isref | clipped) * (int32_t)(c >> 4);
        }
      } else {
        for (uint64_t k = c0; k < c1; k++) {
          const uint32_t c = cigar[k];
          const uint32_t op = c & 0xF;
          if (!(op == OP_S || op == OP_H)) break;
          up -= (int32_t)(c >> 4);
        }
      }
    }
  }
  upos[i] = up;
  score[i] = 0;
}

__device__ __forceinline__ uint32_t first_bytes32(int n) { return n <= 0 ? 0u : (n >= 4 ? 0xFFFFFFFFu : (0xFFFFFFFFu >> (32 - 8 * n))); }

struct ScoreBody {
  static constexpr int NT = FL_THREADS, TILES = 4, RMAX = 1024;
  const uint16_t *__restrict__ flag;
  const uint8_t *__restrict__ qual;
  int32_t *score;
  uint64_t *qbounds;
  int32_t *acc;
  uint32_t *lo;
  uint32_t *hi;
  uint8_t *cand;
  const uint4 *mask;
  uint32_t bad;

  __device__ __forceinline__ void stage(uint32_t g0, uint32_t ng) {
    for (uint32_t k = threadIdx.x; k < ng; k += NT) {
      acc[k] = 0;
      lo[k] = 0xFFFFFFFFu;
      hi[k] = 0u;
      cand[k] = (flag[g0 + k] & (F_UNMAPPED | F_SECONDARY | F_SUPPLEMENTARY)) == 0;
    }
  }
  static __device__ __forceinline__ uint32_t part(uint32_t x, uint32_t s) {
    const uint32_t ge15 = ((x + 0x71717171u) & 0x80808080u) >> 7;
    return __builtin_amdgcn_sad_u8(x & (ge15 * 0xFFu), 0u, s);
  }
  static __device__ __forceinline__ uint32_t gt2(uint32_t x) { return (((x | 0x80808080u) - 0x03030303u) | x) & 0x80808080u; }
  static __device__ __forceinline__ uint32_t ge94(uint32_t x) { return x | (x + 0x22222222u); }
  struct Pre { Chunk ch; uint32_t rl; int nb; int k0; };
  __device__ __forceinline__ bool prefetch(uint32_t rl, int k0, int nb, uint64_t qpos, uint32_t, Pre &p) {
    p.rl = rl; p.nb = nb; p.k0 = k0;
    p.ch.load(qual + qpos);
    return true;
  }
  __device__ __forceinline__ void process(Pre &p) {
    const uint4 mk = mask[p.nb];
    const uint32_t x0 = p.ch.w0 & mk.x, x1 = p.ch.w1 & mk.y, x2 = p.ch.w2 & mk.z, x3 = p.ch.w3 & mk.w;
    const uint64_t glo = (uint64_t)gt2(x0) | ((uint64_t)gt2(x1) << 32);
    const uint64_t ghi = (uint64_t)gt2(x2) | ((uint64_t)gt2(x3) << 32);
    if (glo | ghi) {
      const int first = glo ? (__builtin_ctzll(glo) >> 3) : 8 + (__builtin_ctzll(ghi) >> 3);
      const int last = ghi ? 8 + ((63 - __builtin_clzll(ghi)) >> 3) : ((63 - __builtin_clzll(glo)) >> 3);
      atomicMin(&lo[p.rl], (uint32_t)(p.k0 + first));
      atomicMax(&hi[p.rl], (uint32_t)(p.k0 + last + 1));
    }
    if (!cand[p.rl]) return;
    bad |= (ge94(x0) | ge94(x1) | ge94(x2) | ge94(x3)) & 0x80808080u;
    const uint32_t s = part(x3, part(x2, part(x1, part(x0, 0u))));
    if (s) atomicAdd(&acc[p.rl], (int32_t)s);
  }
  __device__ __forceinline__ void group_end(uint32_t g0, uint32_t ng) {
    for (uint32_t k = threadIdx.x; k < ng; k += NT) {
      score[g0 + k] = acc[k];
      qbounds[g0 + k] = (uint64_t)hi[k] | ((uint64_t)lo[k] << 32);
    }
  }
  __device__ __forceinline__ void slots(uint32_t) {}
  __device__ __forceinline__ void retire() {}
  __device__ __forceinline__ void tile_end(uint32_t, uint64_t) {}
};

__global__ __launch_bounds__(FL_THREADS) void k_score_flat(uint64_t n, const uint64_t *__restrict__ qual_off, const uint8_t *__restrict__ qual,
                                                           uint64_t qual_bytes, const uint32_t *__restrict__ tile_first,
                                                           const uint16_t *__restrict__ flag, int32_t *score, uint64_t *qbounds, uint32_t *err) {
  __shared__ FlatLds<ScoreBody::RMAX> L;
  __shared__ int32_t acc[ScoreBody::RMAX];
  __shared__ uint32_t lo[ScoreBody::RMAX], hi[ScoreBody::RMAX];
  __shared__ uint8_t cand[ScoreBody::RMAX];
  __shared__ uint4 mask[17];
  if (threadIdx.x <= 16) {
    const int nb = (int)threadIdx.x;
    mask[nb] = make_uint4(first_bytes32(nb), first_bytes32(nb - 4), first_bytes32(nb - 8), first_bytes32(nb - 12));
  }
  __syncthreads();
  ScoreBody B{flag, qual, score, qbounds, acc, lo, hi, cand, mask, 0u};
  flat_run(qual_off, n, qual_bytes, tile_first, L, B);
  if (__any(B.bad != 0) && (threadIdx.x & 63) == 0) atomicOr(&err[0], 1u);
}

constexpr int SU_WAVES = 8, SU_MAX_LEN = 250;
__device__ __forceinline__ uint32_t su_gt2(uint32_t x) { return (((x | 0x80808080u) - 0x03030303u) | x) & 0x80808080u; }
template <int R>
__global__ __launch_bounds__(64 * SU_WAVES) void k_score_uniform(uint64_t n, uint32_t L, const uint8_t *__restrict__ qual, const uint16_t *__restrict__ flag,
                                                                 int32_t *__restrict__ score, uint64_t *__restrict__ qbounds, uint32_t *err,
                                                                 uint32_t qstride ,
                                                                 unsigned long long *qmask, const uint16_t *__restrict__ rgid, const uint16_t *__restrict__ rg_cov,
                                                                 uint2 *__restrict__ arecs ) {
  extern __shared__ __attribute__((aligned(16))) uint32_t su_lds[];
  const uint32_t lane = threadIdx.x & 63u, wave = threadIdx.x >> 6;
  const uint32_t tile_bytes = 64u * L, tile_words = tile_bytes / 4u + 4u;
  uint32_t *tile = su_lds + (size_t)wave * tile_words;
  const uint32_t s = lane * L, w0 = s >> 2, skip = s & 3u;
  const uint32_t nw = (skip + L + 3u) >> 2, tail = (skip + L) & 3u;
  const uint32_t m_first = 0xFFFFFFFFu << (8u * skip), m_last = tail ? 0xFFFFFFFFu >> (32u - 8u * tail) : 0xFFFFFFFFu;
  uint32_t bad = 0;
  uint32_t qm[3] = {0, 0, 0};
  const uint64_t ngroups = (n + 63) / 64;
  for (uint64_t g = (uint64_t)blockIdx.x * SU_WAVES + wave; g < ngroups; g += (uint64_t)gridDim.x * SU_WAVES) {
    const uint64_t r0 = g * 64;
    const uint8_t *base = qual + r0 * L;
    const uint64_t have = (n - r0 < 64 ? n - r0 : 64) * (uint64_t)L;
    uint4 v[R];
#pragma unroll
    for (int k = 0; k < R; k++) {
      const uint32_t off = (uint32_t)k * 1024u + lane * 16u;
      v[k] = make_uint4(0u, 0u, 0u, 0u);
      if (off < have) v[k] = *reinterpret_cast<const uint4 *>(base + off);
    }
#pragma unroll
    for (int k = 0; k < R; k++) {
      const uint32_t off = (uint32_t)k * 1024u + lane * 16u;
      if (off < tile_bytes) *reinterpret_cast<uint4 *>(tile + off / 4u) = v[k];
    }
    const uint64_t r = r0 + lane;
    if (r < n) {
      const uint16_t f = flag[r];
      const bool cand = (f & (F_UNMAPPED | F_SECONDARY | F_SUPPLEMENTARY)) == 0;
      const uint16_t rg = arecs ? rgid[r] : (uint16_t)ELP_NIL16;
      const uint32_t *rw = tile + w0;
      uint32_t x = rw[0] & m_first;
      if (nw == 1) x &= m_last;
      constexpr uint32_t NONE = 0xFFFFFFFFu;
      uint32_t sum = ScoreBody::part(x, 0u), orx = x;
      uint32_t kf = su_gt2(x) ? 0u : NONE, kl = 0u;
#pragma unroll 8
      for (uint32_t k = 1; k + 1 < nw; k++) {
        x = rw[k];
        sum = ScoreBody::part(x, sum);
        orx |= x;
        const bool gk = su_gt2(x) != 0u;
        kf = min(kf, gk ? k : NONE);
        kl = gk ? k : kl;
      }
      if (nw > 1) {
        x = rw[nw - 1] & m_last;
        sum = ScoreBody::part(x, sum);
        orx |= x;
        const bool gk = su_gt2(x) != 0u;
        kf = min(kf, gk ? nw - 1 : NONE);
        kl = gk ? nw - 1 : kl;
      }
      uint32_t bd = ScoreBody::ge94(orx) & 0x80808080u;
      if (bd) {
        bd = 0;
        for (uint32_t k = 0; k < nw; k++) {
          uint32_t xw = rw[k];
          if (k == 0) xw &= m_first;
          if (k == nw - 1) xw &= m_last;
          bd |= ScoreBody::ge94(xw);
        }
      }
      uint32_t lo = 0xFFFFFFFFu, hi = 0u;
      if (kf != NONE) {
        uint32_t xf = rw[kf], xl = rw[kl];
        if (kf == 0) xf &= m_first;
        if (kf == nw - 1) xf &= m_last;
        if (kl == 0) xl &= m_first;
        if (kl == nw - 1) xl &= m_last;
        lo = kf * 4u + ((uint32_t)__builtin_ctz(su_gt2(xf)) >> 3) - skip;
        hi = kl * 4u + ((31u - (uint32_t)__builtin_clz(su_gt2(xl))) >> 3) - skip + 1u;
      }
      score[r] = cand ? (int32_t)sum : 0;
      qbounds[r] = (uint64_t)hi | ((uint64_t)lo << 32);
      if (cand) bad |= bd & 0x80808080u;
      if (arecs) arecs[r] = rg == ELP_NIL16 ? make_uint2(AR_NO_RG, 0u) : apply_record(L, (int)L, f, (uint64_t)hi | ((uint64_t)lo << 32), rg_cov[rg]);
      if ((uint32_t)g % qstride == 0) {
        for (uint32_t k = 0; k < nw; k++) {
          const uint32_t vm = (k == 0 ? m_first : 0xFFFFFFFFu) & (k + 1 == nw ? m_last : 0xFFFFFFFFu), xw = rw[k];
#pragma unroll
          for (int b = 0; b < 4; b++) {
            const uint32_t q = (xw >> (8 * b)) & 0xFFu, bit = ((vm >> (8 * b)) & 1u) << (q & 31u), ws = q >> 5;
            qm[0] |= ws == 0 ? bit : 0u;
            qm[1] |= ws == 1 ? bit : 0u;
            qm[2] |= ws == 2 ? bit : 0u;
          }
        }
      }
    }
  }
  if (__any(bad != 0) && lane == 0) atomicOr(&err[0], 1u);
  if (__any((qm[0] | qm[1] | qm[2]) != 0)) {
    for (int d = 32; d >= 1; d >>= 1) {
      qm[0] |= __shfl_xor(qm[0], d, 64);
      qm[1] |= __shfl_xor(qm[1], d, 64);
      qm[2] |= __shfl_xor(qm[2], d, 64);
    }
    if (lane == 0) {
      const unsigned long long lo = (unsigned long long)qm[0] | ((unsigned long long)qm[1] << 32);
      if (lo) atomicOr(&qmask[0], lo);
      if (qm[2]) atomicOr(&qmask[1], (unsigned long long)qm[2]);
    }
  }
}
static bool score_uniform_ok(uint32_t L) {
  if (L < 16 || L > (uint32_t)SU_MAX_LEN) return false;
  if (L % 4u) return true;
  return ((L / 4u) % 4u) != 0;
}
template <int R>
static int score_uniform_launch(elp_ctx *c) {
  const uint32_t L = c->uniform_len;
  const size_t dyn = (size_t)SU_WAVES * ((size_t)64 * L + 16);
  const unsigned per_cu = (unsigned)std::max<size_t>(1, (160 * 1024) / (dyn + 256));
  const uint64_t ngroups = (c->n + 63) / 64;
  const unsigned grid = (unsigned)std::min<uint64_t>((ngroups + SU_WAVES - 1) / SU_WAVES, (uint64_t)c->n_cu * per_cu);
  ELP_HIP(c, hipFuncSetAttribute(reinterpret_cast<const void *>(&k_score_uniform<R>), hipFuncAttributeMaxDynamicSharedMemorySize, (int)dyn));
  uint2 *arecs = nullptr;
  if (L >= 16 && L <= 0x7FFF && c->n_rg > 0) {
    ELP_TRY(ensure(c, c->apply_recs, c->n + 4));
    arecs = c->apply_recs.p;
  }
  const uint32_t qstride = (uint32_t)std::min<uint64_t>(128, std::max<uint64_t>(1, ngroups / 8192));
  ELP_LAUNCH(c, "adapt_score", k_score_uniform<R>, dim3(grid), dim3(64 * SU_WAVES), dyn, c->n, L, (const uint8_t *)c->qual.p, (const uint16_t *)c->flag.p,
             c->score.p, c->qbounds.p, c->adapt_err.p, qstride, reinterpret_cast<unsigned long long *>(c->adapt_err.p + 2), (const uint16_t *)c->rgid.p,
             (const uint16_t *)c->rg_cov.p, arecs);
  c->derived.adapt_sampled = true;
  c->derived.apply_recs_valid = arecs != nullptr;
  c->apply_recs_lmax = (int)L;
  return 0;
}
static int score_uniform(elp_ctx *c) {
  switch ((c->uniform_len + 15u) / 16u) {
#define ELP_SU(R) case R: return score_uniform_launch<R>(c);
    ELP_SU(1) ELP_SU(2) ELP_SU(3) ELP_SU(4) ELP_SU(5) ELP_SU(6) ELP_SU(7) ELP_SU(8) ELP_SU(9) ELP_SU(10) ELP_SU(11) ELP_SU(12) ELP_SU(13) ELP_SU(14)
    ELP_SU(15) ELP_SU(16)
#undef ELP_SU
  }
  return set_error(c, ELP_ERR_ARG, "score_uniform: read length %u", c->uniform_len);
}

__global__ __launch_bounds__(256) void k_qual_present_sample(const uint8_t *__restrict__ qual, uint64_t qual_bytes, uint64_t stride, uint64_t span,
                                                             unsigned long long *qmask) {
  const uint64_t ntiles = (qual_bytes + FL_TILE - 1) / FL_TILE;
  uint32_t m[3] = {0, 0, 0};
  for (uint64_t t = (uint64_t)blockIdx.x * stride; t < ntiles; t += (uint64_t)gridDim.x * stride) {
    const uint64_t tb = t * FL_TILE, te = (tb + span < qual_bytes) ? tb + span : qual_bytes;
    for (uint64_t p = tb + (uint64_t)threadIdx.x * 16; p < te; p += 256 * 16) {
      Chunk ch;
      ch.load(qual + p);
      const int nv = (int)((te - p) < 16 ? (te - p) : 16);
#pragma unroll
      for (int i = 0; i < 16; i++) {
        const uint32_t wv = (i >> 2) == 0 ? ch.w0 : ((i >> 2) == 1 ? ch.w1 : ((i >> 2) == 2 ? ch.w2 : ch.w3));
        const uint32_t q = (wv >> (8 * (i & 3))) & 0xFFu;
        const uint32_t bit = (i < nv) ? (1u << (q & 31u)) : 0u;
        const uint32_t wsel = q >> 5;
        m[0] |= wsel == 0 ? bit : 0u;
        m[1] |= wsel == 1 ? bit : 0u;
        m[2] |= wsel == 2 ? bit : 0u;
      }
    }
  }
  for (int d = 32; d >= 1; d >>= 1) {
    m[0] |= __shfl_xor(m[0], d, 64);
    m[1] |= __shfl_xor(m[1], d, 64);
    m[2] |= __shfl_xor(m[2], d, 64);
  }
  if ((threadIdx.x & 63) == 0) {
    const unsigned long long lo = (unsigned long long)m[0] | ((unsigned long long)m[1] << 32);
    if (lo) atomicOr(&qmask[0], lo);
    if (m[2]) atomicOr(&qmask[1], (unsigned long long)m[2]);
  }
}

__global__ __launch_bounds__(256) void k_flat_index(const uint64_t *__restrict__ qual_off, uint64_t n_reads, uint64_t ntiles,
                                                    uint32_t *__restrict__ tile_first) {
  const uint64_t t = (uint64_t)blockIdx.x * blockDim.x + threadIdx.x;
  if (t > ntiles) return;
  if (t == ntiles) { tile_first[t] = (uint32_t)n_reads; return; }
  const uint64_t x = t * FL_TILE;
  uint64_t lo = 0, hi = n_reads;
  while (lo < hi) {
    const uint64_t mid = lo + (hi - lo) / 2;
    if (qual_off[mid] >= x) hi = mid; else lo = mid + 1;
  }
  tile_first[t] = (uint32_t)lo;
}

int ensure_flat_index(elp_ctx *c) {
  if (c->derived.has_flat_index(c->n, c->qual_bytes)) return 0;
  const uint64_t ntiles = (c->qual_bytes + FL_TILE - 1) / FL_TILE;
  ELP_TRY(ensure(c, c->tile_first, ntiles + 2));
  if (c->n)
    ELP_LAUNCH(c, "flat_index", k_flat_index, dim3(blocks_for(ntiles + 1, 256)), dim3(256), 0, (const uint64_t *)c->qual_off.p, c->n, ntiles,
               c->tile_first.p);
  c->derived.flat_index_n = c->n;
  c->derived.flat_index_bytes = c->qual_bytes;
  return 0;
}

__global__ __launch_bounds__(256) void k_uniform_check(uint64_t n, const uint64_t *__restrict__ qual_off, const uint64_t *__restrict__ seq_off,
                                                       const uint32_t *__restrict__ l_seq, uint64_t len, uint64_t sb, uint64_t seq_front, uint32_t *bad) {
  const uint64_t i = (uint64_t)blockIdx.x * blockDim.x + threadIdx.x;
  bool b = false;
  if (i < n) b = qual_off[i] != i * len || seq_off[i] != seq_front + i * sb || (uint64_t)l_seq[i] != len;
  if (i == n) b = qual_off[n] != n * len || seq_off[n] != seq_front + n * sb;
  if (__any(b) && (threadIdx.x & 63) == 0) atomicOr(bad, 1u);
}
int ensure_uniform_len(elp_ctx *c) {
  if (c->derived.has_uniform(c->n, c->qual_bytes)) return 0;
  c->uniform_len = 0;
  c->derived.uniform_n = c->n;
  c->derived.uniform_bytes = c->qual_bytes;
  if (!c->n || c->qual_bytes % c->n) return 0;
  const uint64_t len = c->qual_bytes / c->n;
  if (len == 0 || len > 0x3FFFFFull) return 0;
  uint32_t *bad = c->err_flag.p + 2;
  ELP_HIP(c, hipMemsetAsync(bad, 0, 4, c->stream));
  ELP_LAUNCH(c, "uniform_check", k_uniform_check, dim3(blocks_for(c->n + 1, 256)), dim3(256), 0, c->n, (const uint64_t *)c->qual_off.p,
             (const uint64_t *)c->seq_off.p, (const uint32_t *)c->l_seq.p, len, (len + 1) / 2, (uint64_t)elp_ctx::SEQ_FRONT, bad);
  uint32_t hb = 0;
  ELP_HIP(c, hipMemcpyAsync(&hb, bad, 4, hipMemcpyDeviceToHost, c->stream));
  ELP_HIP(c, elp::stream_wait(c->stream));
  ELP_HIP(c, hipMemsetAsync(bad, 0, 4, c->stream));
  if (!hb) c->uniform_len = (uint32_t)len;
  return 0;
}

int adapt_quality_error(elp_ctx *c) {
  return set_error(c, ELP_ERR_DATA, "Invalid QUAL character (phred > 93) in a duplicate-marking candidate (reference: log.Panic, filters/mark-duplicates.go:64-66)");
}

static int adapt_resolve(elp_ctx *c) {
  if (!c->derived.adapt_pending) return 0;
  uint32_t w[ADAPT_WORDS];
  ELP_HIP(c, hipMemcpyAsync(w, c->adapt_err.p, sizeof w, hipMemcpyDeviceToHost, c->stream));
  ELP_HIP(c, elp::stream_wait(c->stream));
  adapt_note(c, w);
  return 0;
}
void adapt_note(elp_ctx *c, const uint32_t *words) {
  c->derived.adapt_word_read((words[0] & 1u) != 0);
  if (c->derived.adapt_sampled) {
    c->adapt_qmask[0] = (unsigned long long)words[2] | ((unsigned long long)words[3] << 32);
    c->adapt_qmask[1] = (unsigned long long)words[4] | ((unsigned long long)words[5] << 32);
  }
}
int adapt_begin(elp_ctx *c, int *pos_bits_out) {
  ELP_HIP(c, hipSetDevice(c->device));
  const uint64_t n = c->n;
  ELP_TRY(ensure_flat_index(c));
  ELP_TRY(ensure(c, c->upos, n + 1));
  ELP_TRY(ensure(c, c->score, n + 1));
  ELP_TRY(ensure(c, c->key, n + 1));
  ELP_TRY(ensure(c, c->qbounds, n + 1));
  ELP_TRY(ensure(c, c->adapt_err, ADAPT_WORDS + 2));
  ELP_HIP(c, hipMemsetAsync(c->adapt_err.p, 0, ADAPT_WORDS * sizeof(uint32_t), c->stream));
  c->derived.adapt_begins();
  int pos_bits = 1;
  while (pos_bits < 32 && (c->max_pos >> pos_bits) != 0) pos_bits++;
  int ref_bits = 1;
  while (ref_bits < 32 && (((uint32_t)c->n_ref + 1u) >> ref_bits) != 0) ref_bits++;
  c->key_bits = ref_bits + pos_bits + 1;
  *pos_bits_out = pos_bits;
  return 0;
}
int adapt_scores(elp_ctx *c) {
  const uint64_t n = c->n;
  if (!n) return 0;
  if (!c->qual_bytes) {
    ELP_HIP(c, hipMemsetAsync(c->qbounds.p, 0, n * sizeof(uint64_t), c->stream));
    ELP_HIP(c, hipMemsetAsync(c->score.p, 0, n * sizeof(int32_t), c->stream));
    return 0;
  }
  ELP_TRY(ensure_uniform_len(c));
  if (c->uniform_len && score_uniform_ok(c->uniform_len) && c->tune.score_kernel != 1) {
    ELP_TRY(score_uniform(c));
  } else {
    ELP_HIP(c, hipMemsetAsync(c->score.p, 0, n * sizeof(int32_t), c->stream));
    const unsigned grid = (unsigned)std::min<uint64_t>(flat_steps<ScoreBody>(c->qual_bytes), (uint64_t)c->n_cu * 4);
    ELP_LAUNCH(c, "adapt_score_flat", k_score_flat, dim3(grid), dim3(FL_THREADS), 0, n, (const uint64_t *)c->qual_off.p, (const uint8_t *)c->qual.p,
               c->qual_bytes, (const uint32_t *)c->tile_first.p, (const uint16_t *)c->flag.p, c->score.p, c->qbounds.p, c->adapt_err.p);
  }
  c->derived.adapt_pending = true;
  return 0;
}
int ensure_adapted(elp_ctx *c, bool check_quals) {
  if (c->derived.adapted()) {
    if (check_quals) ELP_TRY(adapt_resolve(c));
    return (check_quals && c->derived.adapt_bad_qual) ? adapt_quality_error(c) : 0;
  }
  int pos_bits = 1;
  ELP_TRY(adapt_begin(c, &pos_bits));
  const uint64_t n = c->n;
  if (n) {
    ELP_LAUNCH(c, "adapt_fixed", k_adapt_fixed, dim3(blocks_for(n, 256)), dim3(256), 0, n, (const int32_t *)c->pos.p, (const int32_t *)c->refid.p,
               (const uint16_t *)c->flag.p, (const uint64_t *)c->cigar_off.p, (const uint32_t *)c->cigar.p, c->upos.p, c->score.p, c->key.p,
               (uint32_t)c->n_ref, pos_bits, (const uint8_t *)c->has_sr.p);
    ELP_TRY(adapt_scores(c));
  }
  c->derived.keys = c->derived.scores = true;
  if (check_quals) ELP_TRY(adapt_resolve(c));
  return (check_quals && c->derived.adapt_bad_qual) ? adapt_quality_error(c) : 0;
}
int ensure_keys(elp_ctx *c) { return c->derived.keys ? 0 : ensure_adapted(c, false); }

int ensure_qual_present(elp_ctx *c, bool exact) {
  if (c->derived.have_qual_present) return 0;
  c->qual_present[0] = c->qual_present[1] = 0;
  if (!exact && c->tune.qual_hint != 1 && c->derived.scores && c->derived.adapt_sampled) {
    ELP_TRY(adapt_resolve(c));
    c->qual_present[0] = c->adapt_qmask[0];
    c->qual_present[1] = c->adapt_qmask[1];
  } else if (c->qual_bytes && (exact || c->tune.qual_hint != 1)) {
    unsigned long long *qm;
    ELP_TRY(scratch(c, 6, 4, &qm));
    ELP_HIP(c, hipMemsetAsync(qm, 0, 16, c->stream));
    const uint64_t ntiles = (c->qual_bytes + FL_TILE - 1) / FL_TILE;
    const uint64_t stride = exact ? 1 : std::min<uint64_t>(16, std::max<uint64_t>(1, ntiles / 2048));
    const unsigned grid = (unsigned)std::min<uint64_t>((ntiles + stride - 1) / stride, 2048);
    ELP_LAUNCH(c, "qual_present_sample", k_qual_present_sample, dim3(grid), dim3(256), 0, (const uint8_t *)c->qual.p, c->qual_bytes, stride,
               (exact || stride == 1) ? FL_TILE : (uint64_t)4096, qm);
    ELP_HIP(c, hipMemcpyAsync(c->qual_present, qm, 16, hipMemcpyDeviceToHost, c->stream));
    ELP_HIP(c, elp::stream_wait(c->stream));
  }
  if (!exact && c->tune.qual_hint_drop >= 0) {
    const int q = c->tune.qual_hint_drop;
    if (q < 64) c->qual_present[0] &= ~(1ull << q);
    else if (q < 128) c->qual_present[1] &= ~(1ull << (q - 64));
  }
  c->derived.have_qual_present = true;
  return 0;
}

struct TieCols {
  const uint64_t *qname_off;
  const uint8_t *qname;
  const uint16_t *flag;
  const uint8_t *mapq;
  const int32_t *next_refid, *pnext, *tlen;
  const uint8_t *rows = nullptr;
  uint32_t rw = 0;
};

__device__ inline bool tie_less(const TieCols &t, uint32_t a, uint32_t b) {
  const uint32_t la = (uint32_t)(t.qname_off[a + 1] - t.qname_off[a]), lb = (uint32_t)(t.qname_off[b + 1] - t.qname_off[b]);
  if (la != 0 && lb != 0) {
    int c = qname_cmp(t.qname, t.qname_off, a, b);
    if (c < 0) return true;
    if (c > 0) return false;
  }
  const uint16_t fa = mod_flag(t.flag[a]), fb = mod_flag(t.flag[b]);
  if (fa < fb) return true;
  if (fa > fb) return false;
  const uint8_t ma = t.mapq[a], mb = t.mapq[b];
  if (ma < mb) return true;
  if (ma > mb) return false;
  if ((t.flag[a] & F_MULTIPLE) && (t.flag[b] & F_MULTIPLE)) {
    const int32_t na = t.next_refid[a], nb = t.next_refid[b];
    if (na < nb) return true;
    if (na > nb) return false;
    const int32_t pa = t.pnext[a], pb = t.pnext[b];
    if (pa < pb) return true;
    if (pa > pb) return false;
  }
  return t.tlen[a] < t.tlen[b];
}

__global__ __launch_bounds__(256) void k_iota(uint32_t *v, uint64_t n) {
  uint64_t i = (uint64_t)blockIdx.x * blockDim.x + threadIdx.x;
  if (i < n) v[i] = (uint32_t)i;
}

struct SortedView {
  const uint64_t *__restrict__ keys;
  const uint32_t *__restrict__ vals;
  uint32_t idx_bits;
  __device__ __forceinline__ uint64_t key(uint64_t i) const { return idx_bits ? keys[i] >> idx_bits : keys[i]; }
  __device__ __forceinline__ uint32_t val(uint64_t i) const { return idx_bits ? (uint32_t)(keys[i] & ((1ull << idx_bits) - 1ull)) : vals[i]; }
};

constexpr int TS_TILES = 32;
__global__ __launch_bounds__(256) void k_tie_scan(uint64_t n, SortedView sv, uint32_t *__restrict__ perm_out, uint32_t *__restrict__ list, uint32_t *list_n,
                                                  uint32_t *__restrict__ bounds) {
  if (blockIdx.x == 0 && threadIdx.x < 4) bounds[threadIdx.x] = 0;
  __shared__ uint32_t lq[TS_TILES * 256];
  __shared__ uint32_t lcount, gbase;
  if (threadIdx.x == 0) lcount = 0;
  __syncthreads();
#pragma unroll 1
  for (int tile = 0; tile < TS_TILES; tile++) {
    const uint64_t i = ((uint64_t)blockIdx.x * TS_TILES + (uint64_t)tile) * 256 + threadIdx.x;
    bool in_run = false;
    if (i < n) {
      const uint64_t w = sv.keys[i], wp = i > 0 ? sv.keys[i - 1] : 0ull, wn = i + 1 < n ? sv.keys[i + 1] : 0ull;
      const uint64_t k = w >> sv.idx_bits, kp = i > 0 ? wp >> sv.idx_bits : ~k, kn = i + 1 < n ? wn >> sv.idx_bits : ~k;
      const uint32_t me = sv.idx_bits ? (uint32_t)(w & ((1ull << sv.idx_bits) - 1ull)) : sv.vals[i];
      in_run = kp == k || kn == k;
      if (!in_run) perm_out[i] = me;
    }
    const unsigned long long mask = __ballot(in_run);
    if (mask) {
      const int lane = threadIdx.x & 63, leader = __ffsll((long long)mask) - 1;
      uint32_t base = 0;
      if (lane == leader) base = atomicAdd(&lcount, (uint32_t)__popcll(mask));
      base = __shfl(base, leader, 64);
      if (in_run) lq[base + (uint32_t)__popcll(mask & ((1ull << lane) - 1ull))] = (uint32_t)i;
    }
  }
  __syncthreads();
  if (threadIdx.x == 0) gbase = lcount ? atomicAdd(list_n, lcount) : 0u;
  __syncthreads();
  for (uint32_t k = threadIdx.x; k < lcount; k += 256) list[gbase + k] = lq[k];
}
__global__ __launch_bounds__(256) void k_tie_small(uint64_t n, SortedView sv, uint32_t *__restrict__ perm_out, uint32_t *__restrict__ bounds ,
                                                   uint32_t bounds_cap, const uint32_t *__restrict__ list, const uint32_t *__restrict__ list_n, TieCols t) {
  const uint64_t j0 = (uint64_t)blockIdx.x * blockDim.x + threadIdx.x;
  if (j0 >= (uint64_t)*list_n) return;
  const uint64_t i = list[j0];
  const uint64_t k = sv.key(i);
  const uint32_t me = sv.val(i);
  uint64_t s = i, e = i + 1;
  bool large = false;
  while (s > 0 && sv.key(s - 1) == k) {
    s--;
    if (i - s >= (uint64_t)TIE_SMALL) { large = true; break; }
  }
  if (!large) {
    while (e < n && sv.key(e) == k) {
      e++;
      if (e - s > (uint64_t)TIE_SMALL) { large = true; break; }
    }
  }
  if (large) {
    perm_out[i] = me;
    if (i == 0 || sv.key(i - 1) != k) { const uint32_t at = atomicAdd(&bounds[0], 1u); if (at < bounds_cap) bounds[4 + at] = (uint32_t)i; }
    if (i + 1 == n || sv.key(i + 1) != k) { const uint32_t at = atomicAdd(&bounds[1], 1u); if (at < bounds_cap) bounds[4 + bounds_cap + at] = (uint32_t)i; }
    return;
  }
  if (e - s == 2) {
    if (i != s) return;
    const uint32_t other = sv.val(s + 1);
    const bool swap = tie_less(t, other, me);
    perm_out[s] = swap ? other : me;
    perm_out[s + 1] = swap ? me : other;
    return;
  }
  uint32_t rank = 0;
  for (uint64_t j = s; j < e; j++) {
    if (j == i) continue;
    const uint32_t other = sv.val(j);
    if (tie_less(t, other, me)) rank++;
    else if (j < i && !tie_less(t, me, other)) rank++;
  }
  perm_out[s + rank] = me;
}

__global__ __launch_bounds__(256) void k_large_fill(uint32_t nu, uint32_t nr, const uint32_t *__restrict__ start, const uint32_t *__restrict__ first,
                                                    SortedView sv, uint32_t *__restrict__ u_pos, uint32_t *__restrict__ u_read,
                                                    uint32_t *__restrict__ u_seg) {
  const uint32_t j = blockIdx.x * blockDim.x + threadIdx.x;
  if (j >= nu) return;
  uint32_t lo = 0, hi = nr;
  while (hi - lo > 1) {
    const uint32_t mid = (lo + hi) >> 1;
    if (first[mid] <= j) lo = mid; else hi = mid;
  }
  const uint32_t pos = start[lo] + (j - first[lo]);
  u_pos[j] = pos;
  u_read[j] = sv.val(pos);
  u_seg[j] = lo + 1u;
}

__device__ inline uint32_t material_byte(const TieCols &t, uint32_t r, uint32_t j, uint32_t maxq, uint32_t m = 0) {
  if (t.rows) return t.rows[(size_t)m * t.rw + j];
  if (j < maxq) {
    const uint64_t o = t.qname_off[r];
    const uint32_t l = (uint32_t)(t.qname_off[r + 1] - o);
    return j < l ? t.qname[o + j] : 0u;
  }
  const uint32_t f = j - maxq;
  const uint16_t fl = t.flag[r];
  if (f < 2) { const uint16_t m = mod_flag(fl); return f == 0 ? (m >> 8) : (m & 0xFF); }
  if (f == 2) return t.mapq[r];
  if (f < 11) {
    if (!(fl & F_MULTIPLE)) return 0u;
    const uint32_t v = (f < 7 ? (uint32_t)t.next_refid[r] : (uint32_t)t.pnext[r]) ^ 0x80000000u;
    const uint32_t b = (f < 7) ? (f - 3) : (f - 7);
    return (v >> (8 * (3 - b))) & 0xFF;
  }
  if (f < 15) {
    const uint32_t v = (uint32_t)t.tlen[r] ^ 0x80000000u;
    return (v >> (8 * (3 - (f - 11)))) & 0xFF;
  }
  return 0u;
}

__global__ __launch_bounds__(256) void k_material_rows(uint32_t nu, const uint32_t *__restrict__ u_read, uint32_t maxq, uint32_t nbytes, uint32_t rw,
                                                       uint8_t *__restrict__ rows, TieCols t ) {
  const uint64_t g = (uint64_t)blockIdx.x * blockDim.x + threadIdx.x;
  const uint32_t per = rw >> 3;
  const uint64_t m = g / per;
  if (m >= nu) return;
  const uint32_t k = (uint32_t)(g - m * per) * 8u, r = u_read[m];
  uint64_t v = 0;
  for (uint32_t i = 0; i < 8; i++)
    if (k + i < nbytes) v |= (uint64_t)material_byte(t, r, k + i, maxq) << (8 * i);
  reinterpret_cast<uint64_t *>(rows + m * rw)[k >> 3] = v;
}

__global__ __launch_bounds__(256) void k_material_live(uint32_t nu, const uint32_t *__restrict__ u_read, uint32_t maxq, uint32_t nbytes,
                                                       uint32_t *live, TieCols t) {
  __shared__ uint32_t acc[elp_ctx::TIE_LIVE_WORDS];
  if (threadIdx.x < elp_ctx::TIE_LIVE_WORDS) acc[threadIdx.x] = 0;
  __syncthreads();
  const uint32_t m = blockIdx.x * blockDim.x + threadIdx.x;
  if (m < nu && t.rows) {
    const uint64_t *a8 = reinterpret_cast<const uint64_t *>(t.rows + (size_t)m * t.rw), *b8 = reinterpret_cast<const uint64_t *>(t.rows);
    for (uint32_t k = 0; k < nbytes; k += 8) {
      uint64_t x = a8[k >> 3] ^ b8[k >> 3];
      if (x) {
        x |= x >> 4; x |= x >> 2; x |= x >> 1;
        x &= 0x0101010101010101ull;
        const uint32_t bits = (uint32_t)((x * 0x0102040810204080ull) >> 56);
        for (uint32_t i = 0; i < 8 && k + i < nbytes; i++)
          if ((bits >> i) & 1u) atomicOr(&acc[(k + i) >> 5], 1u << ((k + i) & 31));
      }
    }
  } else if (m < nu) {
    const uint32_t r = u_read[m], r0 = u_read[0];
    const uint64_t oa = t.qname_off[r], ob = t.qname_off[r0];
    const uint32_t la = (uint32_t)(t.qname_off[r + 1] - oa), lb = (uint32_t)(t.qname_off[r0 + 1] - ob);
    for (uint32_t k = 0; k < maxq; k += 8) {
      const uint64_t a = k < la ? low_bytes(load8(t.qname + oa + k), la - k) : 0ull;
      const uint64_t b = k < lb ? low_bytes(load8(t.qname + ob + k), lb - k) : 0ull;
      uint64_t x = a ^ b;
      if (x) {
        x |= x >> 4; x |= x >> 2; x |= x >> 1;
        x &= 0x0101010101010101ull;
        const uint32_t bits = (uint32_t)((x * 0x0102040810204080ull) >> 56);
        for (uint32_t i = 0; i < 8 && k + i < maxq; i++)
          if ((bits >> i) & 1u) atomicOr(&acc[(k + i) >> 5], 1u << ((k + i) & 31));
      }
    }
    for (uint32_t j = maxq; j < nbytes; j++)
      if (material_byte(t, r, j, maxq) != material_byte(t, r0, j, maxq)) atomicOr(&acc[j >> 5], 1u << (j & 31));
  }
  __syncthreads();
  if (threadIdx.x < elp_ctx::TIE_LIVE_WORDS && acc[threadIdx.x]) atomicOr(&live[threadIdx.x], acc[threadIdx.x]);
}

constexpr int TIE_MAX_PACKED = 96;
struct TiePosList { uint16_t pos[TIE_MAX_PACKED]; uint32_t n; };
__global__ __launch_bounds__(256) void k_material_values(uint32_t nu, const uint32_t *__restrict__ u_read, TiePosList lp, uint32_t maxq,
                                                         uint32_t *vals , TieCols t) {
  __shared__ uint32_t acc[TIE_MAX_PACKED * 8];
  for (uint32_t k = threadIdx.x; k < lp.n * 8; k += blockDim.x) acc[k] = 0;
  __syncthreads();
  for (uint32_t m = blockIdx.x * blockDim.x + threadIdx.x; m < nu; m += gridDim.x * blockDim.x) {
    const uint32_t r = u_read[m];
    for (uint32_t k = 0; k < lp.n; k++) {
      const uint32_t v = material_byte(t, r, lp.pos[k], maxq, m);
      const uint32_t bit = 1u << (v & 31u);
      uint32_t *w = &acc[k * 8 + (v >> 5)];
      if (!(*w & bit)) atomicOr(w, bit);
    }
  }
  __syncthreads();
  for (uint32_t k = threadIdx.x; k < lp.n * 8; k += blockDim.x)
    if (acc[k]) atomicOr(&vals[k], acc[k]);
}
struct TiePacked { uint16_t pos[64]; uint8_t shift[64]; uint8_t slot[64]; uint32_t n; };
__global__ __launch_bounds__(256) void k_material_keys_packed(uint32_t nu, const uint32_t *__restrict__ vals, const uint32_t *__restrict__ u_read,
                                                              TiePacked sel, const uint8_t *__restrict__ lut, uint32_t maxq, uint64_t *__restrict__ keys,
                                                              TieCols t, const uint32_t *__restrict__ u_seg, uint32_t seg_shift) {
  uint32_t j = blockIdx.x * blockDim.x + threadIdx.x;
  if (j >= nu) return;
  const uint32_t mem = vals[j], r = u_read[mem];
  uint64_t k = u_seg ? (uint64_t)u_seg[mem] << seg_shift : 0ull;
  for (uint32_t b = 0; b < sel.n; b++) k |= (uint64_t)lut[(uint32_t)sel.slot[b] * 256u + material_byte(t, r, sel.pos[b], maxq, mem)] << sel.shift[b];
  keys[j] = k;
}

struct TieSel { uint16_t pos[8]; uint32_t n; };
__global__ __launch_bounds__(256) void k_material_keys_sel(uint32_t nu, const uint32_t *__restrict__ vals, const uint32_t *__restrict__ u_read,
                                                           TieSel sel, uint32_t maxq, uint64_t *__restrict__ keys, TieCols t) {
  uint32_t j = blockIdx.x * blockDim.x + threadIdx.x;
  if (j >= nu) return;
  const uint32_t mem = vals[j], r = u_read[mem];
  uint64_t k = 0;
  for (uint32_t b = 0; b < sel.n; b++) k = (k << 8) | material_byte(t, r, sel.pos[b], maxq, mem);
  keys[j] = k;
}

__global__ __launch_bounds__(256) void k_seg_keys(uint32_t nu, const uint32_t *__restrict__ vals, const uint32_t *__restrict__ u_seg_incl,
                                                  uint64_t *__restrict__ keys) {
  uint32_t j = blockIdx.x * blockDim.x + threadIdx.x;
  if (j < nu) keys[j] = (uint64_t)u_seg_incl[vals[j]];
}


__device__ inline int material_cmp(const TieCols &t, uint32_t ma, uint32_t ra, uint32_t mb, uint32_t rb, uint32_t nbytes, uint32_t maxq) {
  if (t.rows) {
    const uint64_t *a8 = reinterpret_cast<const uint64_t *>(t.rows + (size_t)ma * t.rw), *b8 = reinterpret_cast<const uint64_t *>(t.rows + (size_t)mb * t.rw);
    for (uint32_t k = 0; k < nbytes; k += 8) {
      const uint64_t x = a8[k >> 3], y = b8[k >> 3];
      if (x != y) return __builtin_bswap64(x) < __builtin_bswap64(y) ? -1 : 1;
    }
    return 0;
  }
  for (uint32_t j = 0; j < nbytes; j++) {
    const uint32_t x = material_byte(t, ra, j, maxq), y = material_byte(t, rb, j, maxq);
    if (x != y) return x < y ? -1 : 1;
  }
  return 0;
}
constexpr uint32_t LT_CAP = 1024;
__global__ __launch_bounds__(256) void k_large_ties(uint32_t nu, const uint64_t *__restrict__ keys, const uint32_t *__restrict__ vals,
                                                    uint32_t *__restrict__ vals_out, const uint32_t *__restrict__ u_read, uint32_t nbytes, uint32_t maxq,
                                                    uint32_t *over, TieCols t) {
  const uint32_t j = blockIdx.x * blockDim.x + threadIdx.x;
  if (j >= nu) return;
  const uint64_t k = keys[j];
  const uint32_t me = vals[j];
  const bool eq_prev = j > 0 && keys[j - 1] == k, eq_next = j + 1 < nu && keys[j + 1] == k;
  if (!eq_prev && !eq_next) { vals_out[j] = me; return; }
  uint32_t s = j, e = j + 1;
  bool large = false;
  while (s > 0 && keys[s - 1] == k) {
    s--;
    if (j - s >= LT_CAP) { large = true; break; }
  }
  while (!large && e < nu && keys[e] == k) {
    e++;
    if (e - s > LT_CAP) large = true;
  }
  if (large) {
    vals_out[j] = me;
    if (!eq_prev) atomicOr(over, 1u);
    return;
  }
  const uint32_t rme = u_read[me];
  uint32_t rank = 0;
  for (uint32_t i = s; i < e; i++) {
    if (i == j) continue;
    const uint32_t other = vals[i];
    const int c = material_cmp(t, other, u_read[other], me, rme, nbytes, maxq);
    if (c < 0 || (c == 0 && other < me)) rank++;
  }
  vals_out[s + rank] = me;
}

__global__ __launch_bounds__(256) void k_large_scatter(uint32_t nu, const uint32_t *__restrict__ vals_sorted, const uint32_t *__restrict__ u_pos,
                                                       const uint32_t *__restrict__ u_read, uint32_t *__restrict__ perm_out) {
  uint32_t j = blockIdx.x * blockDim.x + threadIdx.x;
  if (j < nu) perm_out[u_pos[j]] = u_read[vals_sorted[j]];
}

static int sort_impl(elp_ctx *c, uint64_t *presorted = nullptr ) {
  const uint64_t n = c->n;
  ELP_TRY(ensure_keys(c));
  ELP_TRY(ensure(c, c->perm, n + 1));
  if (n == 0) { c->derived.set_sorted(false); return 0; }
  uint64_t *kbuf;
  uint32_t *vbuf, *flags;
  ELP_TRY(scratch(c, 0, 2 * n + 8, &kbuf));
  ELP_TRY(scratch(c, 1, 2 * n + 8, &vbuf));
  ELP_TRY(scratch(c, 2, 2 * n + 8, &flags));
  uint64_t *k0 = kbuf, *k1 = kbuf + n;
  uint32_t *v0 = vbuf, *v1 = vbuf + n;
  uint64_t *ks;
  uint32_t *vs = nullptr;
  int idx_bits = 1;
  while (idx_bits < 32 && (n >> idx_bits) != 0) idx_bits++;
  const bool words = c->tune.sort_pairs != 1 && c->key_bits >= 1 && c->key_bits + idx_bits <= 64;
  if (words && presorted) ks = presorted;
  else if (words) ELP_TRY(radix_sort_fused(c, c->key.p, n, c->key_bits, idx_bits, k0, k1, &ks));
  else {
    ProfScope ps(c, "sort_pairs_");
    ELP_TRY(radix_sort_pairs_low(c, k0, v0, k1, v1, n, (c->key_bits + 7) / 8, &ks, &vs, c->key.p, true));
  }
  const SortedView sv{ks, vs, words ? (uint32_t)idx_bits : 0u};
  TieCols t{c->qname_off.p, c->qname.p, c->flag.p, c->mapq.p, c->next_refid.p, c->pnext.p, c->tlen.p};
  const uint32_t bounds_cap = (uint32_t)std::min<uint64_t>(n / TIE_SMALL + 16, (2 * n + 8 - 4) / 2);
  uint32_t *bounds = flags;
  {
    uint32_t *list = (vs == v0) ? v1 : v0, *list_n = c->err_flag.p + 3;
    ELP_HIP(c, hipMemsetAsync(list_n, 0, 4, c->stream));
    ELP_LAUNCH(c, "tie_scan", k_tie_scan, dim3(blocks_for(n, 256 * TS_TILES)), dim3(256), 0, n, sv, c->perm.p, list, list_n, bounds);
    ELP_LAUNCH(c, "tie_small", k_tie_small, dim3(blocks_for(n, 256)), dim3(256), 0, n, sv, c->perm.p, bounds, bounds_cap, (const uint32_t *)list, (const uint32_t *)list_n, t);
    ELP_HIP(c, hipMemsetAsync(list_n, 0, 4, c->stream));
  }
  constexpr uint32_t TIE_HEAD = 256;
  std::vector<uint32_t> hb(4 + 2 * (size_t)TIE_HEAD), starts, ends;
  {
    const uint32_t head = std::min<uint32_t>(TIE_HEAD, bounds_cap);
    ELP_HIP(c, hipMemcpyAsync(hb.data(), bounds, (4 + (size_t)head) * 4, hipMemcpyDeviceToHost, c->stream));
    ELP_HIP(c, hipMemcpyAsync(hb.data() + 4 + TIE_HEAD, bounds + 4 + bounds_cap, (size_t)head * 4, hipMemcpyDeviceToHost, c->stream));
    ELP_HIP(c, elp::stream_wait(c->stream));
  }
  const uint32_t nr = hb[0];
  if (nr != hb[1] || nr > bounds_cap) return set_error(c, ELP_ERR_HIP, "coordinate sort: %u starts and %u ends of long runs (internal)", hb[0], hb[1]);
  uint32_t nu = 0;
  if (nr > 0) {
    starts.resize(nr); ends.resize(nr);
    if (nr <= TIE_HEAD) {
      std::copy(hb.begin() + 4, hb.begin() + 4 + nr, starts.begin());
      std::copy(hb.begin() + 4 + TIE_HEAD, hb.begin() + 4 + TIE_HEAD + nr, ends.begin());
    } else {
      ELP_HIP(c, hipMemcpyAsync(starts.data(), bounds + 4, (size_t)nr * 4, hipMemcpyDeviceToHost, c->stream));
      ELP_HIP(c, hipMemcpyAsync(ends.data(), bounds + 4 + bounds_cap, (size_t)nr * 4, hipMemcpyDeviceToHost, c->stream));
      ELP_HIP(c, elp::stream_wait(c->stream));
    }
    std::sort(starts.begin(), starts.end());
    std::sort(ends.begin(), ends.end());
    std::vector<uint32_t> first(nr + 1);
    uint64_t total = 0;
    for (uint32_t r = 0; r < nr; r++) {
      if (ends[r] < starts[r] || (r + 1 < nr && starts[r + 1] <= ends[r])) return set_error(c, ELP_ERR_HIP, "coordinate sort: long runs overlap (internal)");
      first[r] = (uint32_t)total;
      total += (uint64_t)ends[r] - starts[r] + 1;
    }
    first[nr] = (uint32_t)total;
    nu = (uint32_t)total;
    const uint32_t rw = (c->max_qname_len + 15u + 15u) & ~15u;
    const bool use_rows = (uint64_t)nu * rw <= (512ull << 20);
    const size_t u_words = ((size_t)5 * nu + 2 * (size_t)nr + 64 + 3) & ~(size_t)3;
    uint32_t *u;
    ELP_TRY(scratch(c, 3, u_words + (use_rows ? ((size_t)nu * rw + 64) / 4 : 0), &u));
    uint32_t *u_pos = u, *u_read = u + nu, *u_seg = u + 2 * (size_t)nu, *uv0 = u + 3 * (size_t)nu, *uv1 = u + 4 * (size_t)nu, *d_start = u + 5 * (size_t)nu,
             *d_first = d_start + nr;
    uint64_t *uk;
    ELP_TRY(scratch(c, 4, (size_t)2 * nu + 16, &uk));
    uint64_t *uk0 = uk, *uk1 = uk + nu;
    ELP_HIP(c, hipMemcpyAsync(d_start, starts.data(), (size_t)nr * 4, hipMemcpyHostToDevice, c->stream));
    ELP_HIP(c, hipMemcpyAsync(d_first, first.data(), ((size_t)nr + 1) * 4, hipMemcpyHostToDevice, c->stream));
    ELP_LAUNCH(c, "large_fill", k_large_fill, dim3(blocks_for(nu, 256)), dim3(256), 0, nu, nr, (const uint32_t *)d_start, (const uint32_t *)d_first, sv, u_pos, u_read, u_seg);
    ELP_LAUNCH(c, "iota", k_iota, dim3(blocks_for(nu, 256)), dim3(256), 0, uv0, (uint64_t)nu);
    const uint32_t maxq = c->max_qname_len;
    const uint32_t m_bytes = maxq + 15;
    static_assert(elp_ctx::MAX_QNAME + 15 <= 32 * elp_ctx::TIE_LIVE_WORDS, "live-position bitmap too small");
    ELP_TRY(ensure(c, c->tie_live, elp_ctx::TIE_LIVE_WORDS));
    ELP_HIP(c, hipMemsetAsync(c->tie_live.p, 0, elp_ctx::TIE_LIVE_WORDS * sizeof(uint32_t), c->stream));
    if (use_rows) {
      uint8_t *rows = reinterpret_cast<uint8_t *>(u + u_words);
      ELP_LAUNCH(c, "material_rows", k_material_rows, dim3(blocks_for((uint64_t)nu * (rw >> 3), 256)), dim3(256), 0, nu, (const uint32_t *)u_read, maxq, m_bytes, rw,
                 rows, t);
      t.rows = rows;
      t.rw = rw;
    }
    ELP_LAUNCH(c, "material_live", k_material_live, dim3(blocks_for(nu, 256)), dim3(256), 0, nu, (const uint32_t *)u_read, maxq, m_bytes,
               c->tie_live.p, t);
    uint32_t live[elp_ctx::TIE_LIVE_WORDS];
    ELP_HIP(c, hipMemcpyAsync(live, c->tie_live.p, sizeof live, hipMemcpyDeviceToHost, c->stream));
    ELP_HIP(c, elp::stream_wait(c->stream));
    std::vector<uint16_t> lp;
    for (uint32_t j = 0; j < m_bytes; j++)
      if ((live[j >> 5] >> (j & 31)) & 1u) lp.push_back((uint16_t)j);
    uint32_t *vcur = uv0, *vtmp = uv1;
    bool packed_done = false;
    if (!lp.empty() && lp.size() <= (size_t)TIE_MAX_PACKED) {
      TiePosList pl;
      pl.n = (uint32_t)lp.size();
      for (size_t k = 0; k < lp.size(); k++) pl.pos[k] = lp[k];
      uint32_t *d_vals;
      ELP_TRY(scratch(c, 5, (size_t)TIE_MAX_PACKED * 8 + (size_t)TIE_MAX_PACKED * 64 + 64, &d_vals));
      uint8_t *d_lut = reinterpret_cast<uint8_t *>(d_vals + TIE_MAX_PACKED * 8);
      ELP_HIP(c, hipMemsetAsync(d_vals, 0, (size_t)pl.n * 8 * 4, c->stream));
      ELP_LAUNCH(c, "material_values", k_material_values, dim3(std::min(blocks_for(nu, 256), 1024u)), dim3(256), 0, nu, (const uint32_t *)u_read, pl, maxq, d_vals, t);
      std::vector<uint32_t> hv((size_t)pl.n * 8);
      ELP_HIP(c, hipMemcpyAsync(hv.data(), d_vals, hv.size() * 4, hipMemcpyDeviceToHost, c->stream));
      ELP_HIP(c, elp::stream_wait(c->stream));
      std::vector<uint8_t> lut((size_t)pl.n * 256, 0);
      std::vector<int> bits(pl.n);
      for (uint32_t k = 0; k < pl.n; k++) {
        int rank = 0;
        for (int v = 0; v < 256; v++)
          if ((hv[(size_t)k * 8 + (v >> 5)] >> (v & 31)) & 1u) lut[(size_t)k * 256 + v] = (uint8_t)rank++;
        int b = 1;
        while ((1 << b) < rank) b++;
        bits[k] = b;
      }
      ELP_HIP(c, hipMemcpyAsync(d_lut, lut.data(), lut.size(), hipMemcpyHostToDevice, c->stream));
      int segbits = 0;
      while (nr > 1 && (1u << segbits) <= nr) segbits++;
      if (c->tune.tie_rounds != 1 && segbits + bits[0] <= 64) {
        TiePacked sel;
        memset(&sel, 0, sizeof sel);
        int total = 0, hi = 0;
        while (hi < (int)pl.n && hi < 64 && segbits + total + bits[hi] <= 64) total += bits[hi++];
        int sh = total;
        for (int k = 0; k < hi; k++) {
          sh -= bits[k];
          sel.pos[sel.n] = pl.pos[k]; sel.shift[sel.n] = (uint8_t)sh; sel.slot[sel.n] = (uint8_t)k;
          sel.n++;
        }
        ELP_LAUNCH(c, "material_keys", k_material_keys_packed, dim3(blocks_for(nu, 256)), dim3(256), 0, nu, (const uint32_t *)vcur, (const uint32_t *)u_read,
                   sel, (const uint8_t *)d_lut, maxq, uk0, t, (const uint32_t *)(nr > 1 ? u_seg : nullptr), (uint32_t)total);
        uint64_t *ko;
        uint32_t *vo;
        ELP_TRY(radix_sort_pairs_low(c, uk0, vcur, uk1, vtmp, nu, (segbits + total + 7) / 8, &ko, &vo));
        if (vo != vcur) { vtmp = vcur; vcur = vo; }
        bool settled = hi == (int)pl.n;
        if (!settled) {
          uint32_t *over = c->err_flag.p + 3;
          ELP_LAUNCH(c, "large_ties", k_large_ties, dim3(blocks_for(nu, 256)), dim3(256), 0, nu, (const uint64_t *)ko, (const uint32_t *)vcur, vtmp,
                     (const uint32_t *)u_read, m_bytes, maxq, over, t);
          std::swap(vcur, vtmp);
          ELP_LAUNCH(c, "large_scatter", k_large_scatter, dim3(blocks_for(nu, 256)), dim3(256), 0, nu, (const uint32_t *)vcur, (const uint32_t *)u_pos,
                     (const uint32_t *)u_read, c->perm.p);
          uint32_t h_over = 0;
          ELP_HIP(c, hipMemcpyAsync(&h_over, over, 4, hipMemcpyDeviceToHost, c->stream));
          ELP_HIP(c, elp::stream_wait(c->stream));
          settled = h_over == 0;
          if (!settled) {
            ELP_HIP(c, hipMemsetAsync(over, 0, 4, c->stream));
            ELP_LAUNCH(c, "iota", k_iota, dim3(blocks_for(nu, 256)), dim3(256), 0, uv0, (uint64_t)nu);
            vcur = uv0; vtmp = uv1;
          }
        } else {
          ELP_LAUNCH(c, "large_scatter", k_large_scatter, dim3(blocks_for(nu, 256)), dim3(256), 0, nu, (const uint32_t *)vcur, (const uint32_t *)u_pos,
                     (const uint32_t *)u_read, c->perm.p);
        }
        if (settled) {
          c->radix_check_pending = true;
          c->derived.set_sorted(false);
          return 0;
        }
      }
      for (int hi = (int)pl.n; hi > 0;) {
        TiePacked sel;
        memset(&sel, 0, sizeof sel);
        int total = 0, lo = hi;
        while (lo > 0 && total + bits[lo - 1] <= 64 && hi - lo < 64) { lo--; total += bits[lo]; }
        int sh = total;
        for (int k = lo; k < hi; k++) {
          sh -= bits[k];
          sel.pos[sel.n] = pl.pos[k]; sel.shift[sel.n] = (uint8_t)sh; sel.slot[sel.n] = (uint8_t)k;
          sel.n++;
        }
        ELP_LAUNCH(c, "material_keys", k_material_keys_packed, dim3(blocks_for(nu, 256)), dim3(256), 0, nu, (const uint32_t *)vcur, (const uint32_t *)u_read,
                   sel, (const uint8_t *)d_lut, maxq, uk0, t, (const uint32_t *)nullptr, 0u);
        uint64_t *ko;
        uint32_t *vo;
        ELP_TRY(radix_sort_pairs_low(c, uk0, vcur, uk1, vtmp, nu, (total + 7) / 8, &ko, &vo));
        if (vo != vcur) { vtmp = vcur; vcur = vo; }
        hi = lo;
      }
      packed_done = true;
    }
    for (size_t hi = packed_done ? 0 : lp.size(); hi > 0;) {
      const size_t lo = hi >= 8 ? hi - 8 : 0;
      TieSel sel;
      sel.n = (uint32_t)(hi - lo);
      for (size_t b = 0; b < 8; b++) sel.pos[b] = b < sel.n ? lp[lo + b] : 0;
      ELP_LAUNCH(c, "material_keys", k_material_keys_sel, dim3(blocks_for(nu, 256)), dim3(256), 0, nu, (const uint32_t *)vcur,
                 (const uint32_t *)u_read, sel, maxq, uk0, t);
      uint64_t *ko;
      uint32_t *vo;
      ELP_TRY(radix_sort_pairs_low(c, uk0, vcur, uk1, vtmp, nu, (int)sel.n, &ko, &vo));
      if (vo != vcur) { vtmp = vcur; vcur = vo; }
      hi = lo;
    }
    if (nr > 1) ELP_LAUNCH(c, "seg_keys", k_seg_keys, dim3(blocks_for(nu, 256)), dim3(256), 0, nu, (const uint32_t *)vcur, (const uint32_t *)u_seg, uk0);
    if (nr > 1) {
      uint64_t *ko;
      uint32_t *vo;
      ELP_TRY(radix_sort_pairs(c, uk0, vcur, uk1, vtmp, nu, &ko, &vo));
      if (vo != vcur) { vtmp = vcur; vcur = vo; }
    }
    ELP_LAUNCH(c, "large_scatter", k_large_scatter, dim3(blocks_for(nu, 256)), dim3(256), 0, nu, (const uint32_t *)vcur, (const uint32_t *)u_pos,
               (const uint32_t *)u_read, c->perm.p);
  }
  c->radix_check_pending = true;
  c->derived.set_sorted(false);
  return 0;
}

}

namespace elp {
static int sort_on_side(elp_ctx *c) {
  ELP_TRY(ensure_keys(c));
  ELP_TRY(ensure(c, c->perm, c->n + 1));
  elp_ctx *s = nullptr;
  ELP_TRY(side_lane(c, 1, &s));
  s->n = c->n; s->n_sr = c->n_sr; s->n_filtered = c->n_filtered; s->key_bits = c->key_bits; s->max_qname_len = c->max_qname_len; s->max_pos = c->max_pos;
  s->n_ref = c->n_ref;
  s->derived = elp::Derived{};
  s->derived.keys = true;
  s->key.p = c->key.p; s->flag.p = c->flag.p; s->mapq.p = c->mapq.p; s->next_refid.p = c->next_refid.p; s->pnext.p = c->pnext.p; s->tlen.p = c->tlen.p;
  s->qname_off.p = c->qname_off.p; s->qname.p = c->qname.p; s->has_sr.p = c->has_sr.p;
  s->perm.p = c->perm.p; s->perm.cap = c->perm.cap;
  int ib = 1;
  while (ib < 32 && (c->n >> ib) != 0) ib++;
  uint64_t *pre = (c->presort_ks && c->derived.presorted && c->presort_n == c->n && c->presort_idx_bits == ib && c->tune.sort_pairs != 1) ? c->presort_ks : nullptr;
  c->derived.drop_presort();
  int rc = sort_impl(s, pre);
  s->key.p = nullptr; s->flag.p = nullptr; s->mapq.p = nullptr; s->next_refid.p = nullptr; s->pnext.p = nullptr; s->tlen.p = nullptr;
  s->qname_off.p = nullptr; s->qname.p = nullptr; s->has_sr.p = nullptr;
  s->perm.p = nullptr; s->perm.cap = 0;
  if (rc == 0) rc = radix_check(s);
  if (rc != 0) {
    (void)elp::stream_wait(s->stream);
    c->err = s->err;
    return rc;
  }
  ELP_TRY(side_join(c, 1));
  c->derived.set_sorted(false);
  return 0;
}
}

namespace elp {
int sort_presort(elp_ctx *c) {
  const uint64_t n = c->n;
  c->derived.drop_presort();
  if (!c->sort_ahead || n < 2 || !c->derived.keys || c->tune.sort_pairs == 1) return 0;
  int idx_bits = 1;
  while (idx_bits < 32 && (n >> idx_bits) != 0) idx_bits++;
  if (c->key_bits < 1 || c->key_bits + idx_bits > 64) return 0;
  elp_ctx *s = nullptr;
  ELP_TRY(side_lane(c, 1, &s));
  s->n = n; s->key_bits = c->key_bits;
  const int tile_saved = s->tune.radix_tile;
  if (!s->tune.radix_tile) s->tune.radix_tile = c->tune.presort_tile >= 1 && c->tune.presort_tile <= 3 ? c->tune.presort_tile : 2;
  uint64_t *kbuf, *ks = nullptr;
  int rc = scratch(s, 0, 2 * n + 8, &kbuf);
  if (rc == 0) rc = radix_sort_fused(s, c->key.p, n, c->key_bits, idx_bits, kbuf, kbuf + n, &ks);
  s->tune.radix_tile = tile_saved;
  if (rc != 0) { c->err = s->err; return rc; }
  c->presort_ks = ks; c->presort_n = n; c->presort_idx_bits = idx_bits; c->derived.presorted = true;
  return 0;
}
}

extern "C" int elp_sort_ahead(elp_ctx *c, int on) {
  if (!c) return ELP_ERR_ARG;
  c->sort_ahead = on != 0;
  if (!on) c->derived.drop_presort();
  return 0;
}

extern "C" int elp_sort_coordinate(elp_ctx *c) {
  if (!c) return ELP_ERR_ARG;
  ELP_HIP(c, hipSetDevice(c->device));
  c->derived.drop_sorted();
  return elp::sort_on_side(c);
}
```

Before: 2314.

## Move large-tie sort planning on device to remove host round-trips

Adds a device kernel that plans large tie groups and a combined material-rows/live-byte kernel. A last-block LUT builder computes value ranks, bit widths and the packed key layout into a device descriptor. Radix passes take a per-digit device count stride, so the packed sort runs without the host reading live masks or value histograms and uploading LUTs in between. The goal is to cut synchronous D2H/H2D round-trips and host LUT construction on the tie-break path. In exchange there is more device-side control logic and a pinned mailbox per side lane.

```diff
diff --git a/elprep_amd/csrc/common.hpp b/elprep_amd/csrc/common.hpp
--- a/elprep_amd/csrc/common.hpp
+++ b/elprep_amd/csrc/common.hpp
@@ -403,7 +403,8 @@
 };
 int radix_sort_pairs_low(elp_ctx *c, uint64_t *keys, uint32_t *vals, uint64_t *keys_tmp, uint32_t *vals_tmp, uint64_t n, int ndigits,
                          uint64_t **keys_out, uint32_t **vals_out, const uint64_t *first_src = nullptr, bool identity_vals = false,
-                         const uint32_t *n_dev = nullptr , RadixBounds bnd = RadixBounds{});
+                         const uint32_t *n_dev = nullptr , RadixBounds bnd = RadixBounds{},
+                         int n_dev_stride = 0 );
 int exclusive_scan_u32(elp_ctx *c, const uint32_t *in, uint32_t *out, uint64_t n, uint32_t *total_host );
 int ensure_adapted(elp_ctx *c, bool check_quals = true);
 int ensure_keys(elp_ctx *c);
diff --git a/elprep_amd/csrc/ctx.hip b/elprep_amd/csrc/ctx.hip
--- a/elprep_amd/csrc/ctx.hip
+++ b/elprep_amd/csrc/ctx.hip
@@ -303,6 +303,8 @@
       (void)elp::stream_wait(c->side[lane]->stream);
       for (auto &p : c->side[lane]->prof_pending) { (void)hipEventDestroy(p.a); (void)hipEventDestroy(p.b); }
       (void)hipStreamDestroy(c->side[lane]->stream);
+      if (c->side[lane]->mail) (void)hipHostFree(c->side[lane]->mail);
+      if (c->side[lane]->mail_ev) (void)hipEventDestroy(c->side[lane]->mail_ev);
       delete c->side[lane];
       c->side[lane] = nullptr;
     }
diff --git a/elprep_amd/csrc/radix.hip b/elprep_amd/csrc/radix.hip
--- a/elprep_amd/csrc/radix.hip
+++ b/elprep_amd/csrc/radix.hip
@@ -377,7 +377,8 @@
 }
 
 int radix_sort_pairs_low(elp_ctx *c, uint64_t *keys, uint32_t *vals, uint64_t *keys_tmp, uint32_t *vals_tmp, uint64_t n, int ndigits,
-                         uint64_t **keys_out, uint32_t **vals_out, const uint64_t *first_src, bool identity_vals, const uint32_t *n_dev, RadixBounds bnd) {
+                         uint64_t **keys_out, uint32_t **vals_out, const uint64_t *first_src, bool identity_vals, const uint32_t *n_dev, RadixBounds bnd,
+                         int n_dev_stride) {
   *keys_out = keys;
   *vals_out = vals;
   if ((ndigits <= 0 || (n < 2 && !n_dev)) && !first_src && !identity_vals) return 0;
@@ -399,8 +400,8 @@
     ELP_TRY(radix_next_epoch(c));
     const uint64_t *kin = (d == 0 && first_src) ? first_src : ksrc;
     const uint32_t *vin = (d == 0 && identity_vals) ? nullptr : vsrc;
-    ELP_TRY(radix_scatter_launch(c, n, kin, vin, kdst, vdst, 8 * d, (const unsigned long long *)(ghist + d * 256), ticket + d, n_dev,
-                                 d == ndigits - 1 ? bnd : RadixBounds{}));
+    ELP_TRY(radix_scatter_launch(c, n, kin, vin, kdst, vdst, 8 * d, (const unsigned long long *)(ghist + d * 256), ticket + d,
+                                 n_dev ? n_dev + (size_t)d * n_dev_stride : nullptr, d == ndigits - 1 ? bnd : RadixBounds{}));
     std::swap(ksrc, kdst);
     std::swap(vsrc, vdst);
   }
diff --git a/elprep_amd/csrc/sort.hip b/elprep_amd/csrc/sort.hip
--- a/elprep_amd/csrc/sort.hip
+++ b/elprep_amd/csrc/sort.hip
@@ -598,9 +598,38 @@
   perm_out[s + rank] = me;
 }
 
+constexpr uint32_t LP_COUNT = 0;
+constexpr uint32_t LP_FLAGS = 2;
+constexpr uint32_t LP_DONE = 3;
+constexpr uint32_t LP_NSTART = 4, LP_NEND = 5;
+constexpr uint32_t LP_HEAD = 8;
+constexpr uint32_t LP_VALS = 16;
+__global__ __launch_bounds__(256) void k_large_plan(uint64_t n, SortedView sv, const uint32_t *__restrict__ bounds, uint32_t bounds_cap, uint32_t *plan,
+                                                    uint32_t *__restrict__ d_start, uint32_t *__restrict__ d_first) {
+  const uint32_t ns = bounds[0], ne = bounds[1];
+  if (blockIdx.x == 0 && threadIdx.x == 0) {
+    plan[LP_NSTART] = ns;
+    plan[LP_NEND] = ne;
+    if (ns != ne || ns > bounds_cap) atomicOr(&plan[LP_FLAGS], 1u);
+  }
+  const uint32_t nr = ns < bounds_cap ? ns : bounds_cap;
+  for (uint32_t r = blockIdx.x * blockDim.x + threadIdx.x; r < nr; r += gridDim.x * blockDim.x) {
+    const uint64_t s = bounds[4 + r];
+    const uint64_t k = sv.key(s);
+    uint64_t lo = s + TIE_SMALL, hi = n;
+    while (hi - lo > 1) {
+      const uint64_t mid = lo + (hi - lo) / 2;
+      if (sv.key(mid) == k) lo = mid; else hi = mid;
+    }
+    const unsigned long long old = atomicAdd(reinterpret_cast<unsigned long long *>(plan + LP_COUNT), (1ull << 32) | (hi - s));
+    d_start[old >> 32] = (uint32_t)s;
+    d_first[old >> 32] = (uint32_t)old;
+  }
+}
+
 __global__ __launch_bounds__(256) void k_large_fill(uint32_t nu, uint32_t nr, const uint32_t *__restrict__ start, const uint32_t *__restrict__ first,
                                                     SortedView sv, uint32_t *__restrict__ u_pos, uint32_t *__restrict__ u_read,
-                                                    uint32_t *__restrict__ u_seg) {
+                                                    uint32_t *__restrict__ u_seg, uint32_t *__restrict__ iota) {
   const uint32_t j = blockIdx.x * blockDim.x + threadIdx.x;
   if (j >= nu) return;
   uint32_t lo = 0, hi = nr;
@@ -612,6 +641,7 @@
   u_pos[j] = pos;
   u_read[j] = sv.val(pos);
   u_seg[j] = lo + 1u;
+  iota[j] = j;
 }
 
 __device__ inline uint32_t material_byte(const TieCols &t, uint32_t r, uint32_t j, uint32_t maxq, uint32_t m = 0) {
@@ -638,52 +668,58 @@
   return 0u;
 }
 
-__global__ __launch_bounds__(256) void k_material_rows(uint32_t nu, const uint32_t *__restrict__ u_read, uint32_t maxq, uint32_t nbytes, uint32_t rw,
-                                                       uint8_t *__restrict__ rows, TieCols t ) {
+__device__ __forceinline__ uint32_t nonzero_bytes(uint64_t x) {
+  x |= x >> 4; x |= x >> 2; x |= x >> 1;
+  x &= 0x0101010101010101ull;
+  return (uint32_t)((x * 0x0102040810204080ull) >> 56);
+}
+
+constexpr uint32_t TIE_ROW_MAX = (elp_ctx::MAX_QNAME + 15u + 15u) & ~15u;
+__global__ __launch_bounds__(256) void k_material_rows_live(uint32_t nu, const uint32_t *__restrict__ u_read, uint32_t maxq, uint32_t nbytes, uint32_t rw,
+                                                            uint8_t *__restrict__ rows, uint32_t *live, TieCols t ) {
+  __shared__ uint64_t row0[TIE_ROW_MAX / 8];
+  __shared__ uint32_t acc[elp_ctx::TIE_LIVE_WORDS];
+  const uint32_t per = rw >> 3;
+  if (threadIdx.x < elp_ctx::TIE_LIVE_WORDS) acc[threadIdx.x] = 0;
+  const uint32_t r0 = u_read[0];
+  for (uint32_t w = threadIdx.x; w < per; w += blockDim.x) {
+    uint64_t v = 0;
+    for (uint32_t i = 0; i < 8; i++)
+      if (w * 8u + i < nbytes) v |= (uint64_t)material_byte(t, r0, w * 8u + i, maxq) << (8 * i);
+    row0[w] = v;
+  }
+  __syncthreads();
   const uint64_t g = (uint64_t)blockIdx.x * blockDim.x + threadIdx.x;
-  const uint32_t per = rw >> 3;
   const uint64_t m = g / per;
-  if (m >= nu) return;
-  const uint32_t k = (uint32_t)(g - m * per) * 8u, r = u_read[m];
-  uint64_t v = 0;
-  for (uint32_t i = 0; i < 8; i++)
-    if (k + i < nbytes) v |= (uint64_t)material_byte(t, r, k + i, maxq) << (8 * i);
-  reinterpret_cast<uint64_t *>(rows + m * rw)[k >> 3] = v;
+  if (m < nu) {
+    const uint32_t w = (uint32_t)(g - m * per), k = w * 8u, r = u_read[m];
+    uint64_t v = 0;
+    for (uint32_t i = 0; i < 8; i++)
+      if (k + i < nbytes) v |= (uint64_t)material_byte(t, r, k + i, maxq) << (8 * i);
+    reinterpret_cast<uint64_t *>(rows + m * rw)[w] = v;
+    const uint32_t bits = nonzero_bytes(v ^ row0[w]);
+    if (bits) atomicOr(&acc[k >> 5], bits << (k & 31));
+  }
+  __syncthreads();
+  if (threadIdx.x < elp_ctx::TIE_LIVE_WORDS && acc[threadIdx.x]) atomicOr(&live[threadIdx.x], acc[threadIdx.x]);
 }
 
 __global__ __launch_bounds__(256) void k_material_live(uint32_t nu, const uint32_t *__restrict__ u_read, uint32_t maxq, uint32_t nbytes,
-                                                       uint32_t *live, TieCols t) {
+                                                       uint32_t *live, TieCols t ) {
   __shared__ uint32_t acc[elp_ctx::TIE_LIVE_WORDS];
   if (threadIdx.x < elp_ctx::TIE_LIVE_WORDS) acc[threadIdx.x] = 0;
   __syncthreads();
   const uint32_t m = blockIdx.x * blockDim.x + threadIdx.x;
-  if (m < nu && t.rows) {
-    const uint64_t *a8 = reinterpret_cast<const uint64_t *>(t.rows + (size_t)m * t.rw), *b8 = reinterpret_cast<const uint64_t *>(t.rows);
-    for (uint32_t k = 0; k < nbytes; k += 8) {
-      uint64_t x = a8[k >> 3] ^ b8[k >> 3];
-      if (x) {
-        x |= x >> 4; x |= x >> 2; x |= x >> 1;
-        x &= 0x0101010101010101ull;
-        const uint32_t bits = (uint32_t)((x * 0x0102040810204080ull) >> 56);
-        for (uint32_t i = 0; i < 8 && k + i < nbytes; i++)
-          if ((bits >> i) & 1u) atomicOr(&acc[(k + i) >> 5], 1u << ((k + i) & 31));
-      }
-    }
-  } else if (m < nu) {
+  if (m < nu) {
     const uint32_t r = u_read[m], r0 = u_read[0];
     const uint64_t oa = t.qname_off[r], ob = t.qname_off[r0];
     const uint32_t la = (uint32_t)(t.qname_off[r + 1] - oa), lb = (uint32_t)(t.qname_off[r0 + 1] - ob);
     for (uint32_t k = 0; k < maxq; k += 8) {
       const uint64_t a = k < la ? low_bytes(load8(t.qname + oa + k), la - k) : 0ull;
       const uint64_t b = k < lb ? low_bytes(load8(t.qname + ob + k), lb - k) : 0ull;
-      uint64_t x = a ^ b;
-      if (x) {
-        x |= x >> 4; x |= x >> 2; x |= x >> 1;
-        x &= 0x0101010101010101ull;
-        const uint32_t bits = (uint32_t)((x * 0x0102040810204080ull) >> 56);
-        for (uint32_t i = 0; i < 8 && k + i < maxq; i++)
-          if ((bits >> i) & 1u) atomicOr(&acc[(k + i) >> 5], 1u << ((k + i) & 31));
-      }
+      const uint32_t bits = nonzero_bytes(a ^ b);
+      for (uint32_t i = 0; i < 8 && k + i < maxq; i++)
+        if ((bits >> i) & 1u) atomicOr(&acc[(k + i) >> 5], 1u << ((k + i) & 31));
     }
     for (uint32_t j = maxq; j < nbytes; j++)
       if (material_byte(t, r, j, maxq) != material_byte(t, r0, j, maxq)) atomicOr(&acc[j >> 5], 1u << (j & 31));
@@ -693,33 +729,110 @@
 }
 
 constexpr int TIE_MAX_PACKED = 96;
-struct TiePosList { uint16_t pos[TIE_MAX_PACKED]; uint32_t n; };
-__global__ __launch_bounds__(256) void k_material_values(uint32_t nu, const uint32_t *__restrict__ u_read, TiePosList lp, uint32_t maxq,
-                                                         uint32_t *vals , TieCols t) {
+struct TiePacked { uint16_t pos[64]; uint8_t shift[64]; uint8_t slot[64]; uint32_t n; uint32_t seg_shift; };
+struct TieDesc {
+  TiePacked sel;
+  uint32_t n_live;
+  uint32_t settled;
+  uint32_t npass;
+  uint32_t pass_n[8];
+  uint16_t pos[TIE_MAX_PACKED];
+  uint8_t bits[TIE_MAX_PACKED];
+};
+static_assert(sizeof(TiePacked) % 4 == 0 && sizeof(TieDesc) % 4 == 0, "copied as words");
+
+__global__ __launch_bounds__(256) void k_material_values_lut(uint32_t nu, const uint32_t *__restrict__ u_read, const uint32_t *__restrict__ live, uint32_t maxq,
+                                                             uint32_t *vals , uint8_t *__restrict__ lut, TieDesc *desc,
+                                                             uint32_t *done, uint32_t *over, uint32_t segbits, TieCols t) {
   __shared__ uint32_t acc[TIE_MAX_PACKED * 8];
-  for (uint32_t k = threadIdx.x; k < lp.n * 8; k += blockDim.x) acc[k] = 0;
-  __syncthreads();
+  __shared__ uint16_t lpos[TIE_MAX_PACKED];
+  __shared__ uint8_t lbits[TIE_MAX_PACKED];
+  __shared__ uint32_t nl_s, last_s;
+  if (threadIdx.x < elp_ctx::TIE_LIVE_WORDS) {
+    uint32_t at = 0;
+    for (uint32_t w = 0; w < threadIdx.x; w++) at += (uint32_t)__popc(live[w]);
+    uint32_t m = live[threadIdx.x];
+    if (threadIdx.x == elp_ctx::TIE_LIVE_WORDS - 1) nl_s = at + (uint32_t)__popc(m);
+    while (m) {
+      const uint32_t b = (uint32_t)__ffs((int)m) - 1u;
+      m &= m - 1u;
+      if (at < (uint32_t)TIE_MAX_PACKED) lpos[at] = (uint16_t)(threadIdx.x * 32u + b);
+      at++;
+    }
+  }
+  for (uint32_t k = threadIdx.x; k < (uint32_t)TIE_MAX_PACKED * 8; k += blockDim.x) acc[k] = 0;
+  __syncthreads();
+  const uint32_t nl = nl_s;
+  if (nl > (uint32_t)TIE_MAX_PACKED) {
+    if (blockIdx.x == 0 && threadIdx.x == 0) {
+      desc->sel.n = 0; desc->sel.seg_shift = 0; desc->n_live = nl; desc->settled = 0; desc->npass = 0;
+      for (int d = 0; d < 8; d++) desc->pass_n[d] = 0;
+      atomicOr(over, 2u);
+    }
+    return;
+  }
   for (uint32_t m = blockIdx.x * blockDim.x + threadIdx.x; m < nu; m += gridDim.x * blockDim.x) {
     const uint32_t r = u_read[m];
-    for (uint32_t k = 0; k < lp.n; k++) {
-      const uint32_t v = material_byte(t, r, lp.pos[k], maxq, m);
+    for (uint32_t k = 0; k < nl; k++) {
+      const uint32_t v = material_byte(t, r, lpos[k], maxq, m);
       const uint32_t bit = 1u << (v & 31u);
       uint32_t *w = &acc[k * 8 + (v >> 5)];
       if (!(*w & bit)) atomicOr(w, bit);
     }
   }
   __syncthreads();
-  for (uint32_t k = threadIdx.x; k < lp.n * 8; k += blockDim.x)
+  for (uint32_t k = threadIdx.x; k < nl * 8; k += blockDim.x)
     if (acc[k]) atomicOr(&vals[k], acc[k]);
-}
-struct TiePacked { uint16_t pos[64]; uint8_t shift[64]; uint8_t slot[64]; uint32_t n; };
+  __threadfence();
+  __syncthreads();
+  if (threadIdx.x == 0) last_s = atomicAdd(done, 1u) == gridDim.x - 1u ? 1u : 0u;
+  __syncthreads();
+  if (!last_s) return;
+  __threadfence();
+  for (uint32_t k = threadIdx.x; k < nl; k += blockDim.x) {
+    uint32_t rank = 0;
+    for (uint32_t w = 0; w < 8; w++) {
+      const uint32_t m = __hip_atomic_load(&vals[k * 8 + w], __ATOMIC_RELAXED, __HIP_MEMORY_SCOPE_AGENT);
+      for (uint32_t b = 0; b < 32; b++) {
+        const uint32_t present = (m >> b) & 1u;
+        lut[k * 256u + w * 32u + b] = (uint8_t)(present ? rank : 0u);
+        rank += present;
+      }
+    }
+    uint32_t b = 1;
+    while ((1u << b) < rank) b++;
+    lbits[k] = (uint8_t)b;
+  }
+  __syncthreads();
+  if (threadIdx.x == 0) {
+    uint32_t total = 0, hi = 0;
+    while (hi < nl && hi < 64u && segbits + total + lbits[hi] <= 64u) total += lbits[hi++];
+    uint32_t sh = total;
+    for (uint32_t k = 0; k < hi; k++) {
+      sh -= lbits[k];
+      desc->sel.pos[k] = lpos[k]; desc->sel.shift[k] = (uint8_t)sh; desc->sel.slot[k] = (uint8_t)k;
+    }
+    desc->sel.n = hi;
+    desc->sel.seg_shift = total;
+    desc->n_live = nl;
+    desc->settled = hi == nl ? 1u : 0u;
+    const uint32_t npass = (segbits + total + 7u) / 8u;
+    desc->npass = npass;
+    for (uint32_t d = 0; d < 8; d++) desc->pass_n[d] = d < npass ? nu : 0u;
+    for (uint32_t k = 0; k < nl; k++) { desc->pos[k] = lpos[k]; desc->bits[k] = lbits[k]; }
+  }
+}
+
 __global__ __launch_bounds__(256) void k_material_keys_packed(uint32_t nu, const uint32_t *__restrict__ vals, const uint32_t *__restrict__ u_read,
-                                                              TiePacked sel, const uint8_t *__restrict__ lut, uint32_t maxq, uint64_t *__restrict__ keys,
-                                                              TieCols t, const uint32_t *__restrict__ u_seg, uint32_t seg_shift) {
+                                                              const TiePacked *__restrict__ selp, const uint8_t *__restrict__ lut, uint32_t maxq,
+                                                              uint64_t *__restrict__ keys, TieCols t, const uint32_t *__restrict__ u_seg) {
+  __shared__ TiePacked sel;
+  for (uint32_t i = threadIdx.x; i < sizeof(TiePacked) / 4; i += blockDim.x) reinterpret_cast<uint32_t *>(&sel)[i] = reinterpret_cast<const uint32_t *>(selp)[i];
+  __syncthreads();
   uint32_t j = blockIdx.x * blockDim.x + threadIdx.x;
   if (j >= nu) return;
   const uint32_t mem = vals[j], r = u_read[mem];
-  uint64_t k = u_seg ? (uint64_t)u_seg[mem] << seg_shift : 0ull;
+  uint64_t k = u_seg ? (uint64_t)u_seg[mem] << sel.seg_shift : 0ull;
   for (uint32_t b = 0; b < sel.n; b++) k |= (uint64_t)lut[(uint32_t)sel.slot[b] * 256u + material_byte(t, r, sel.pos[b], maxq, mem)] << sel.shift[b];
   keys[j] = k;
 }
@@ -758,15 +871,20 @@
   return 0;
 }
 constexpr uint32_t LT_CAP = 1024;
-__global__ __launch_bounds__(256) void k_large_ties(uint32_t nu, const uint64_t *__restrict__ keys, const uint32_t *__restrict__ vals,
-                                                    uint32_t *__restrict__ vals_out, const uint32_t *__restrict__ u_read, uint32_t nbytes, uint32_t maxq,
-                                                    uint32_t *over, TieCols t) {
+__global__ __launch_bounds__(256) void k_large_ties(uint32_t nu, const uint64_t *__restrict__ keys0, const uint64_t *__restrict__ keys1,
+                                                    const uint32_t *__restrict__ vals0, const uint32_t *__restrict__ vals1, const TieDesc *__restrict__ desc,
+                                                    const uint32_t *__restrict__ u_read, const uint32_t *__restrict__ u_pos, uint32_t *__restrict__ perm_out,
+                                                    uint32_t nbytes, uint32_t maxq, uint32_t *over, TieCols t) {
   const uint32_t j = blockIdx.x * blockDim.x + threadIdx.x;
-  if (j >= nu) return;
+  if (j >= nu || desc->n_live > (uint32_t)TIE_MAX_PACKED) return;
+  const bool odd = (desc->npass & 1u) != 0;
+  const uint64_t *__restrict__ keys = odd ? keys1 : keys0;
+  const uint32_t *__restrict__ vals = odd ? vals1 : vals0;
   const uint64_t k = keys[j];
   const uint32_t me = vals[j];
+  const uint32_t rme = u_read[me];
   const bool eq_prev = j > 0 && keys[j - 1] == k, eq_next = j + 1 < nu && keys[j + 1] == k;
-  if (!eq_prev && !eq_next) { vals_out[j] = me; return; }
+  if ((!eq_prev && !eq_next) || desc->settled) { perm_out[u_pos[j]] = rme; return; }
   uint32_t s = j, e = j + 1;
   bool large = false;
   while (s > 0 && keys[s - 1] == k) {
@@ -778,11 +896,10 @@
     if (e - s > LT_CAP) large = true;
   }
   if (large) {
-    vals_out[j] = me;
+    perm_out[u_pos[j]] = rme;
     if (!eq_prev) atomicOr(over, 1u);
     return;
   }
-  const uint32_t rme = u_read[me];
   uint32_t rank = 0;
   for (uint32_t i = s; i < e; i++) {
     if (i == j) continue;
@@ -790,7 +907,7 @@
     const int c = material_cmp(t, other, u_read[other], me, rme, nbytes, maxq);
     if (c < 0 || (c == 0 && other < me)) rank++;
   }
-  vals_out[s + rank] = me;
+  perm_out[u_pos[s + rank]] = rme;
 }
 
 __global__ __launch_bounds__(256) void k_large_scatter(uint32_t nu, const uint32_t *__restrict__ vals_sorted, const uint32_t *__restrict__ u_pos,
@@ -826,6 +943,20 @@
   TieCols t{c->qname_off.p, c->qname.p, c->flag.p, c->mapq.p, c->next_refid.p, c->pnext.p, c->tlen.p};
   const uint32_t bounds_cap = (uint32_t)std::min<uint64_t>(n / TIE_SMALL + 16, (2 * n + 8 - 4) / 2);
   uint32_t *bounds = flags;
+  constexpr size_t LP_ZERO = LP_VALS + (size_t)TIE_MAX_PACKED * 8, LP_LUT = LP_ZERO, LP_DESC = LP_LUT + (size_t)TIE_MAX_PACKED * 64,
+                   LP_SEL = LP_DESC + (sizeof(TieDesc) + 15) / 16 * 4, SEL_WORDS = (sizeof(TiePacked) + 15) / 16 * 4, SEL_SLOTS = 14,
+                   LP_RUNS = LP_SEL + SEL_SLOTS * SEL_WORDS;
+  static_assert(16 + SEL_SLOTS * SEL_WORDS <= 1024, "the key layouts of the many-rounds path go through the mailbox page");
+  uint32_t *plan;
+  ELP_TRY(scratch(c, 5, LP_RUNS + 2 * (size_t)bounds_cap + 16, &plan));
+  uint32_t *d_vals = plan + LP_VALS, *d_start = plan + LP_RUNS, *d_first = d_start + bounds_cap;
+  uint8_t *d_lut = reinterpret_cast<uint8_t *>(plan + LP_LUT);
+  TieDesc *d_desc = reinterpret_cast<TieDesc *>(plan + LP_DESC);
+  static_assert(elp_ctx::MAX_QNAME + 15 <= 32 * elp_ctx::TIE_LIVE_WORDS, "live-position bitmap too small");
+  ELP_TRY(ensure(c, c->tie_live, elp_ctx::TIE_LIVE_WORDS));
+  ELP_TRY(mailbox(c));
+  ELP_HIP(c, hipMemsetAsync(plan, 0, LP_ZERO * sizeof(uint32_t), c->stream));
+  ELP_HIP(c, hipMemsetAsync(c->tie_live.p, 0, elp_ctx::TIE_LIVE_WORDS * sizeof(uint32_t), c->stream));
   {
     uint32_t *list = (vs == v0) ? v1 : v0, *list_n = c->err_flag.p + 3;
     ELP_HIP(c, hipMemsetAsync(list_n, 0, 4, c->stream));
@@ -833,176 +964,108 @@
     ELP_LAUNCH(c, "tie_small", k_tie_small, dim3(blocks_for(n, 256)), dim3(256), 0, n, sv, c->perm.p, bounds, bounds_cap, (const uint32_t *)list, (const uint32_t *)list_n, t);
     ELP_HIP(c, hipMemsetAsync(list_n, 0, 4, c->stream));
   }
-  constexpr uint32_t TIE_HEAD = 256;
-  std::vector<uint32_t> hb(4 + 2 * (size_t)TIE_HEAD), starts, ends;
-  {
-    const uint32_t head = std::min<uint32_t>(TIE_HEAD, bounds_cap);
-    ELP_HIP(c, hipMemcpyAsync(hb.data(), bounds, (4 + (size_t)head) * 4, hipMemcpyDeviceToHost, c->stream));
-    ELP_HIP(c, hipMemcpyAsync(hb.data() + 4 + TIE_HEAD, bounds + 4 + bounds_cap, (size_t)head * 4, hipMemcpyDeviceToHost, c->stream));
-    ELP_HIP(c, elp::stream_wait(c->stream));
-  }
-  const uint32_t nr = hb[0];
-  if (nr != hb[1] || nr > bounds_cap) return set_error(c, ELP_ERR_HIP, "coordinate sort: %u starts and %u ends of long runs (internal)", hb[0], hb[1]);
-  uint32_t nu = 0;
+  ELP_LAUNCH(c, "large_plan", k_large_plan, dim3(std::min(blocks_for(bounds_cap, 256), 1024u)), dim3(256), 0, n, sv, (const uint32_t *)bounds, bounds_cap, plan,
+             d_start, d_first);
+  ELP_HIP(c, hipMemcpyAsync(c->mail, plan, LP_HEAD * sizeof(uint32_t), hipMemcpyDeviceToHost, c->stream));
+  uint32_t ew[4];
+  ELP_TRY(fetch_err(c, ew));
+  const uint32_t nu = c->mail[LP_COUNT], nr = c->mail[LP_COUNT + 1];
+  if ((c->mail[LP_FLAGS] & 1u) || nr > bounds_cap || nu > n)
+    return set_error(c, ELP_ERR_HIP, "coordinate sort: %u starts and %u ends of long runs (internal)", c->mail[LP_NSTART], c->mail[LP_NEND]);
   if (nr > 0) {
-    starts.resize(nr); ends.resize(nr);
-    if (nr <= TIE_HEAD) {
-      std::copy(hb.begin() + 4, hb.begin() + 4 + nr, starts.begin());
-      std::copy(hb.begin() + 4 + TIE_HEAD, hb.begin() + 4 + TIE_HEAD + nr, ends.begin());
-    } else {
-      ELP_HIP(c, hipMemcpyAsync(starts.data(), bounds + 4, (size_t)nr * 4, hipMemcpyDeviceToHost, c->stream));
-      ELP_HIP(c, hipMemcpyAsync(ends.data(), bounds + 4 + bounds_cap, (size_t)nr * 4, hipMemcpyDeviceToHost, c->stream));
-      ELP_HIP(c, elp::stream_wait(c->stream));
-    }
-    std::sort(starts.begin(), starts.end());
-    std::sort(ends.begin(), ends.end());
-    std::vector<uint32_t> first(nr + 1);
-    uint64_t total = 0;
-    for (uint32_t r = 0; r < nr; r++) {
-      if (ends[r] < starts[r] || (r + 1 < nr && starts[r + 1] <= ends[r])) return set_error(c, ELP_ERR_HIP, "coordinate sort: long runs overlap (internal)");
-      first[r] = (uint32_t)total;
-      total += (uint64_t)ends[r] - starts[r] + 1;
-    }
-    first[nr] = (uint32_t)total;
-    nu = (uint32_t)total;
     const uint32_t rw = (c->max_qname_len + 15u + 15u) & ~15u;
     const bool use_rows = (uint64_t)nu * rw <= (512ull << 20);
-    const size_t u_words = ((size_t)5 * nu + 2 * (size_t)nr + 64 + 3) & ~(size_t)3;
+    const size_t u_words = ((size_t)5 * nu + 64 + 3) & ~(size_t)3;
     uint32_t *u;
     ELP_TRY(scratch(c, 3, u_words + (use_rows ? ((size_t)nu * rw + 64) / 4 : 0), &u));
-    uint32_t *u_pos = u, *u_read = u + nu, *u_seg = u + 2 * (size_t)nu, *uv0 = u + 3 * (size_t)nu, *uv1 = u + 4 * (size_t)nu, *d_start = u + 5 * (size_t)nu,
-             *d_first = d_start + nr;
+    uint32_t *u_pos = u, *u_read = u + nu, *u_seg = u + 2 * (size_t)nu, *uv0 = u + 3 * (size_t)nu, *uv1 = u + 4 * (size_t)nu;
     uint64_t *uk;
     ELP_TRY(scratch(c, 4, (size_t)2 * nu + 16, &uk));
     uint64_t *uk0 = uk, *uk1 = uk + nu;
-    ELP_HIP(c, hipMemcpyAsync(d_start, starts.data(), (size_t)nr * 4, hipMemcpyHostToDevice, c->stream));
-    ELP_HIP(c, hipMemcpyAsync(d_first, first.data(), ((size_t)nr + 1) * 4, hipMemcpyHostToDevice, c->stream));
-    ELP_LAUNCH(c, "large_fill", k_large_fill, dim3(blocks_for(nu, 256)), dim3(256), 0, nu, nr, (const uint32_t *)d_start, (const uint32_t *)d_first, sv, u_pos, u_read, u_seg);
-    ELP_LAUNCH(c, "iota", k_iota, dim3(blocks_for(nu, 256)), dim3(256), 0, uv0, (uint64_t)nu);
+    ELP_LAUNCH(c, "large_fill", k_large_fill, dim3(blocks_for(nu, 256)), dim3(256), 0, nu, nr, (const uint32_t *)d_start, (const uint32_t *)d_first, sv, u_pos, u_read,
+               u_seg, uv0);
     const uint32_t maxq = c->max_qname_len;
     const uint32_t m_bytes = maxq + 15;
-    static_assert(elp_ctx::MAX_QNAME + 15 <= 32 * elp_ctx::TIE_LIVE_WORDS, "live-position bitmap too small");
-    ELP_TRY(ensure(c, c->tie_live, elp_ctx::TIE_LIVE_WORDS));
-    ELP_HIP(c, hipMemsetAsync(c->tie_live.p, 0, elp_ctx::TIE_LIVE_WORDS * sizeof(uint32_t), c->stream));
     if (use_rows) {
       uint8_t *rows = reinterpret_cast<uint8_t *>(u + u_words);
-      ELP_LAUNCH(c, "material_rows", k_material_rows, dim3(blocks_for((uint64_t)nu * (rw >> 3), 256)), dim3(256), 0, nu, (const uint32_t *)u_read, maxq, m_bytes, rw,
-                 rows, t);
+      ELP_LAUNCH(c, "material_rows", k_material_rows_live, dim3(blocks_for((uint64_t)nu * (rw >> 3), 256)), dim3(256), 0, nu, (const uint32_t *)u_read, maxq, m_bytes,
+                 rw, rows, c->tie_live.p, t);
       t.rows = rows;
       t.rw = rw;
-    }
-    ELP_LAUNCH(c, "material_live", k_material_live, dim3(blocks_for(nu, 256)), dim3(256), 0, nu, (const uint32_t *)u_read, maxq, m_bytes,
-               c->tie_live.p, t);
-    uint32_t live[elp_ctx::TIE_LIVE_WORDS];
-    ELP_HIP(c, hipMemcpyAsync(live, c->tie_live.p, sizeof live, hipMemcpyDeviceToHost, c->stream));
+    } else {
+      ELP_LAUNCH(c, "material_live", k_material_live, dim3(blocks_for(nu, 256)), dim3(256), 0, nu, (const uint32_t *)u_read, maxq, m_bytes, c->tie_live.p, t);
+    }
+    int segbits = 0;
+    while (nr > 1 && (1u << segbits) <= nr) segbits++;
+    uint32_t *over = c->err_flag.p + 3;
+    ELP_LAUNCH(c, "material_values", k_material_values_lut, dim3(std::min(blocks_for(nu, 256), 1024u)), dim3(256), 0, nu, (const uint32_t *)u_read,
+               (const uint32_t *)c->tie_live.p, maxq, d_vals, d_lut, d_desc, plan + LP_DONE, over, (uint32_t)segbits, t);
+    if (c->tune.tie_rounds != 1) {
+      ELP_LAUNCH(c, "material_keys", k_material_keys_packed, dim3(blocks_for(nu, 256)), dim3(256), 0, nu, (const uint32_t *)uv0, (const uint32_t *)u_read,
+                 (const TiePacked *)&d_desc->sel, (const uint8_t *)d_lut, maxq, uk0, t, (const uint32_t *)(nr > 1 ? u_seg : nullptr));
+      uint64_t *ko;
+      uint32_t *vo;
+      ELP_TRY(radix_sort_pairs_low(c, uk0, uv0, uk1, uv1, nu, 8, &ko, &vo, nullptr, false, (const uint32_t *)d_desc->pass_n, RadixBounds{}, 1));
+      ELP_LAUNCH(c, "large_ties", k_large_ties, dim3(blocks_for(nu, 256)), dim3(256), 0, nu, (const uint64_t *)uk0, (const uint64_t *)uk1, (const uint32_t *)uv0,
+                 (const uint32_t *)uv1, (const TieDesc *)d_desc, (const uint32_t *)u_read, (const uint32_t *)u_pos, c->perm.p, m_bytes, maxq, over, t);
+      ELP_TRY(fetch_err(c, ew));
+      if (ew[3] == 0) {
+        c->derived.set_sorted(false);
+        return 0;
+      }
+      ELP_HIP(c, hipMemsetAsync(over, 0, 4, c->stream));
+      ELP_LAUNCH(c, "iota", k_iota, dim3(blocks_for(nu, 256)), dim3(256), 0, uv0, (uint64_t)nu);
+    }
+    TieDesc hd;
+    ELP_HIP(c, hipMemcpyAsync(&hd, d_desc, sizeof hd, hipMemcpyDeviceToHost, c->stream));
     ELP_HIP(c, elp::stream_wait(c->stream));
-    std::vector<uint16_t> lp;
-    for (uint32_t j = 0; j < m_bytes; j++)
-      if ((live[j >> 5] >> (j & 31)) & 1u) lp.push_back((uint16_t)j);
+    if (c->tune.tie_rounds == 1 && hd.n_live > (uint32_t)TIE_MAX_PACKED) ELP_HIP(c, hipMemsetAsync(over, 0, 4, c->stream));
     uint32_t *vcur = uv0, *vtmp = uv1;
-    bool packed_done = false;
-    if (!lp.empty() && lp.size() <= (size_t)TIE_MAX_PACKED) {
-      TiePosList pl;
-      pl.n = (uint32_t)lp.size();
-      for (size_t k = 0; k < lp.size(); k++) pl.pos[k] = lp[k];
-      uint32_t *d_vals;
-      ELP_TRY(scratch(c, 5, (size_t)TIE_MAX_PACKED * 8 + (size_t)TIE_MAX_PACKED * 64 + 64, &d_vals));
-      uint8_t *d_lut = reinterpret_cast<uint8_t *>(d_vals + TIE_MAX_PACKED * 8);
-      ELP_HIP(c, hipMemsetAsync(d_vals, 0, (size_t)pl.n * 8 * 4, c->stream));
-      ELP_LAUNCH(c, "material_values", k_material_values, dim3(std::min(blocks_for(nu, 256), 1024u)), dim3(256), 0, nu, (const uint32_t *)u_read, pl, maxq, d_vals, t);
-      std::vector<uint32_t> hv((size_t)pl.n * 8);
-      ELP_HIP(c, hipMemcpyAsync(hv.data(), d_vals, hv.size() * 4, hipMemcpyDeviceToHost, c->stream));
-      ELP_HIP(c, elp::stream_wait(c->stream));
-      std::vector<uint8_t> lut((size_t)pl.n * 256, 0);
-      std::vector<int> bits(pl.n);
-      for (uint32_t k = 0; k < pl.n; k++) {
-        int rank = 0;
-        for (int v = 0; v < 256; v++)
-          if ((hv[(size_t)k * 8 + (v >> 5)] >> (v & 31)) & 1u) lut[(size_t)k * 256 + v] = (uint8_t)rank++;
-        int b = 1;
-        while ((1 << b) < rank) b++;
-        bits[k] = b;
-      }
-      ELP_HIP(c, hipMemcpyAsync(d_lut, lut.data(), lut.size(), hipMemcpyHostToDevice, c->stream));
-      int segbits = 0;
-      while (nr > 1 && (1u << segbits) <= nr) segbits++;
-      if (c->tune.tie_rounds != 1 && segbits + bits[0] <= 64) {
-        TiePacked sel;
-        memset(&sel, 0, sizeof sel);
-        int total = 0, hi = 0;
-        while (hi < (int)pl.n && hi < 64 && segbits + total + bits[hi] <= 64) total += bits[hi++];
-        int sh = total;
-        for (int k = 0; k < hi; k++) {
-          sh -= bits[k];
-          sel.pos[sel.n] = pl.pos[k]; sel.shift[sel.n] = (uint8_t)sh; sel.slot[sel.n] = (uint8_t)k;
-          sel.n++;
-        }
-        ELP_LAUNCH(c, "material_keys", k_material_keys_packed, dim3(blocks_for(nu, 256)), dim3(256), 0, nu, (const uint32_t *)vcur, (const uint32_t *)u_read,
-                   sel, (const uint8_t *)d_lut, maxq, uk0, t, (const uint32_t *)(nr > 1 ? u_seg : nullptr), (uint32_t)total);
-        uint64_t *ko;
-        uint32_t *vo;
-        ELP_TRY(radix_sort_pairs_low(c, uk0, vcur, uk1, vtmp, nu, (segbits + total + 7) / 8, &ko, &vo));
-        if (vo != vcur) { vtmp = vcur; vcur = vo; }
-        bool settled = hi == (int)pl.n;
-        if (!settled) {
-          uint32_t *over = c->err_flag.p + 3;
-          ELP_LAUNCH(c, "large_ties", k_large_ties, dim3(blocks_for(nu, 256)), dim3(256), 0, nu, (const uint64_t *)ko, (const uint32_t *)vcur, vtmp,
-                     (const uint32_t *)u_read, m_bytes, maxq, over, t);
-          std::swap(vcur, vtmp);
-          ELP_LAUNCH(c, "large_scatter", k_large_scatter, dim3(blocks_for(nu, 256)), dim3(256), 0, nu, (const uint32_t *)vcur, (const uint32_t *)u_pos,
-                     (const uint32_t *)u_read, c->perm.p);
-          uint32_t h_over = 0;
-          ELP_HIP(c, hipMemcpyAsync(&h_over, over, 4, hipMemcpyDeviceToHost, c->stream));
-          ELP_HIP(c, elp::stream_wait(c->stream));
-          settled = h_over == 0;
-          if (!settled) {
-            ELP_HIP(c, hipMemsetAsync(over, 0, 4, c->stream));
-            ELP_LAUNCH(c, "iota", k_iota, dim3(blocks_for(nu, 256)), dim3(256), 0, uv0, (uint64_t)nu);
-            vcur = uv0; vtmp = uv1;
-          }
-        } else {
-          ELP_LAUNCH(c, "large_scatter", k_large_scatter, dim3(blocks_for(nu, 256)), dim3(256), 0, nu, (const uint32_t *)vcur, (const uint32_t *)u_pos,
-                     (const uint32_t *)u_read, c->perm.p);
-        }
-        if (settled) {
-          c->radix_check_pending = true;
-          c->derived.set_sorted(false);
-          return 0;
-        }
-      }
-      for (int hi = (int)pl.n; hi > 0;) {
-        TiePacked sel;
-        memset(&sel, 0, sizeof sel);
+    if (hd.n_live <= (uint32_t)TIE_MAX_PACKED) {
+      uint32_t slot = 0;
+      for (int hi = (int)hd.n_live; hi > 0;) {
+        if (slot >= SEL_SLOTS) return set_error(c, ELP_ERR_HIP, "coordinate sort: more tie-break rounds than key layouts (internal)");
+        TiePacked *sel = reinterpret_cast<TiePacked *>(c->mail + 16 + slot * SEL_WORDS);
+        memset(sel, 0, sizeof *sel);
         int total = 0, lo = hi;
-        while (lo > 0 && total + bits[lo - 1] <= 64 && hi - lo < 64) { lo--; total += bits[lo]; }
+        while (lo > 0 && total + hd.bits[lo - 1] <= 64 && hi - lo < 64) { lo--; total += hd.bits[lo]; }
         int sh = total;
         for (int k = lo; k < hi; k++) {
-          sh -= bits[k];
-          sel.pos[sel.n] = pl.pos[k]; sel.shift[sel.n] = (uint8_t)sh; sel.slot[sel.n] = (uint8_t)k;
-          sel.n++;
+          sh -= hd.bits[k];
+          sel->pos[sel->n] = hd.pos[k]; sel->shift[sel->n] = (uint8_t)sh; sel->slot[sel->n] = (uint8_t)k;
+          sel->n++;
         }
+        TiePacked *d_sel = reinterpret_cast<TiePacked *>(plan + LP_SEL + slot * SEL_WORDS);
+        ELP_HIP(c, hipMemcpyAsync(d_sel, sel, sizeof *sel, hipMemcpyHostToDevice, c->stream));
         ELP_LAUNCH(c, "material_keys", k_material_keys_packed, dim3(blocks_for(nu, 256)), dim3(256), 0, nu, (const uint32_t *)vcur, (const uint32_t *)u_read,
-                   sel, (const uint8_t *)d_lut, maxq, uk0, t, (const uint32_t *)nullptr, 0u);
+                   (const TiePacked *)d_sel, (const uint8_t *)d_lut, maxq, uk0, t, (const uint32_t *)nullptr);
         uint64_t *ko;
         uint32_t *vo;
         ELP_TRY(radix_sort_pairs_low(c, uk0, vcur, uk1, vtmp, nu, (total + 7) / 8, &ko, &vo));
         if (vo != vcur) { vtmp = vcur; vcur = vo; }
         hi = lo;
+        slot++;
       }
-      packed_done = true;
-    }
-    for (size_t hi = packed_done ? 0 : lp.size(); hi > 0;) {
-      const size_t lo = hi >= 8 ? hi - 8 : 0;
-      TieSel sel;
-      sel.n = (uint32_t)(hi - lo);
-      for (size_t b = 0; b < 8; b++) sel.pos[b] = b < sel.n ? lp[lo + b] : 0;
-      ELP_LAUNCH(c, "material_keys", k_material_keys_sel, dim3(blocks_for(nu, 256)), dim3(256), 0, nu, (const uint32_t *)vcur,
-                 (const uint32_t *)u_read, sel, maxq, uk0, t);
-      uint64_t *ko;
-      uint32_t *vo;
-      ELP_TRY(radix_sort_pairs_low(c, uk0, vcur, uk1, vtmp, nu, (int)sel.n, &ko, &vo));
-      if (vo != vcur) { vtmp = vcur; vcur = vo; }
-      hi = lo;
+    } else {
+      uint32_t live[elp_ctx::TIE_LIVE_WORDS];
+      ELP_HIP(c, hipMemcpyAsync(live, c->tie_live.p, sizeof live, hipMemcpyDeviceToHost, c->stream));
+      ELP_HIP(c, elp::stream_wait(c->stream));
+      std::vector<uint16_t> lp;
+      for (uint32_t j = 0; j < m_bytes; j++)
+        if ((live[j >> 5] >> (j & 31)) & 1u) lp.push_back((uint16_t)j);
+      for (size_t hi = lp.size(); hi > 0;) {
+        const size_t lo = hi >= 8 ? hi - 8 : 0;
+        TieSel sel;
+        sel.n = (uint32_t)(hi - lo);
+        for (size_t b = 0; b < 8; b++) sel.pos[b] = b < sel.n ? lp[lo + b] : 0;
+        ELP_LAUNCH(c, "material_keys", k_material_keys_sel, dim3(blocks_for(nu, 256)), dim3(256), 0, nu, (const uint32_t *)vcur,
+                   (const uint32_t *)u_read, sel, maxq, uk0, t);
+        uint64_t *ko;
+        uint32_t *vo;
+        ELP_TRY(radix_sort_pairs_low(c, uk0, vcur, uk1, vtmp, nu, (int)sel.n, &ko, &vo));
+        if (vo != vcur) { vtmp = vcur; vcur = vo; }
+        hi = lo;
+      }
     }
     if (nr > 1) ELP_LAUNCH(c, "seg_keys", k_seg_keys, dim3(blocks_for(nu, 256)), dim3(256), 0, nu, (const uint32_t *)vcur, (const uint32_t *)u_seg, uk0);
     if (nr > 1) {
@@ -1013,8 +1076,8 @@
     }
     ELP_LAUNCH(c, "large_scatter", k_large_scatter, dim3(blocks_for(nu, 256)), dim3(256), 0, nu, (const uint32_t *)vcur, (const uint32_t *)u_pos,
                (const uint32_t *)u_read, c->perm.p);
-  }
-  c->radix_check_pending = true;
+    c->radix_check_pending = true;
+  }
   c->derived.set_sorted(false);
   return 0;
 }
```

New measurement: 2306. No clear change (-0.3%).
